# ServiceFoundation/partisan

Measured on AMD Instinct MI355X. Metric: simulated node-rounds/sec (+ msgs/sec), 1M-node HyParView+Plumtree, higher is better.
Workload: dtype u32

## Files before the change

### include/partisan_gpu_sim.h

```cpp
#ifndef PARTISAN_GPU_SIM_H
#define PARTISAN_GPU_SIM_H

#include <stddef.h>
#include <stdint.h>

#ifdef __cplusplus
extern "C" {
#endif

#define PSIM_ABI_VERSION 12

#define PSIM_OK 0
#define PSIM_EINVAL -1
#define PSIM_ENOMEM -2
#define PSIM_EDEVICE -3
#define PSIM_ESTATE -4
#define PSIM_ERANGE -5
#define PSIM_ECOMM -6
#define PSIM_EUNSUPPORTED -7
#define PSIM_ECAPACITY -8

enum psim_msg_type {
    PSIM_MSG_JOIN = 0,
    PSIM_MSG_FORWARD_JOIN = 1,
// ... 309 lines not shown
    uint64_t relays[PSIM_RELAY_CASES];
    uint64_t refused[PSIM_RELAY_CASES];
    uint64_t expired[PSIM_RELAY_CASES];
    uint64_t restarts[PSIM_RELAY_CASES];
    uint64_t in_flight[PSIM_RELAY_CASES];
    uint64_t levels[PSIM_RELAY_CASES];
    uint64_t peak[PSIM_RELAY_CASES];
    uint64_t reserved[8];
} psim_relay_reach;

typedef struct psim_handle psim_handle;

void psim_default_config(psim_config *cfg);
int psim_create(const psim_config *cfg, psim_handle **out);
void psim_destroy(psim_handle *h);
const char *psim_strerror(int code);
int psim_abi_version(void);

int psim_join(psim_handle *h, const uint32_t *nodes, const uint32_t *contacts, size_t n);
int psim_crash(psim_handle *h, const uint32_t *nodes, size_t n);
int psim_revive(psim_handle *h, const uint32_t *nodes, size_t n);
int psim_leave(psim_handle *h, const uint32_t *nodes, size_t n);
int psim_leave_node(psim_handle *h, const uint32_t *actors, const uint32_t *targets, size_t n);
#define PSIM_PARTITION_MAX 254
int psim_set_partition(psim_handle *h, const uint8_t *group, size_t n);
int psim_set_bucket_table(psim_handle *h, const uint8_t *buckets, size_t n);
int psim_set_phash_table(psim_handle *h, const uint32_t *phash, size_t n);
int psim_clear_partition(psim_handle *h);
#define PSIM_OMIT_SEND 0
#define PSIM_OMIT_RECEIVE 1
int psim_set_omission(psim_handle *h, int kind, const uint32_t *src, const uint32_t *dst, size_t n, int on);
int psim_set_faulted(psim_handle *h, const uint32_t *nodes, size_t n, int on);
int psim_clear_faults(psim_handle *h);
int psim_broadcast(psim_handle *h, uint32_t root, uint32_t msg_id);

int psim_step(psim_handle *h, uint32_t n_rounds, psim_round_stats *stats);

int psim_get_nodes(psim_handle *h, uint32_t first, uint32_t count, psim_node_view *out);
int psim_get_round(psim_handle *h, uint64_t *round);
int psim_get_strategy_nodes(psim_handle *h, uint32_t first, uint32_t count, psim_strategy_view *out);
int psim_get_member_bits(psim_handle *h, uint32_t node, uint32_t *words, size_t n_words);
int psim_get_delivery(psim_handle *h, uint32_t first, uint32_t count, uint8_t *have, uint32_t *round,
                      uint32_t *hop);
int psim_get_histograms(psim_handle *h, psim_histograms *out);
int psim_get_strategy_histograms(psim_handle *h, psim_strategy_histograms *out);
int psim_get_graph_metrics(psim_handle *h, const uint32_t *sources, size_t n_sources, uint32_t max_levels,
                           psim_graph_metrics *out);
int psim_get_tree_metrics(psim_handle *h, uint32_t root, uint32_t max_levels, psim_tree_metrics *out);
int psim_get_resilience(psim_handle *h, const psim_failure_case *cases, size_t n_cases, uint64_t fail_seed,
                        uint32_t max_levels, psim_resilience *out);
int psim_get_gossip_reach(psim_handle *h, const psim_gossip_case *cases, size_t n_cases, uint64_t fail_seed,
                          uint32_t max_levels, psim_gossip_reach *out);
int psim_get_relay_reach(psim_handle *h, const psim_relay_case *cases, size_t n_cases, uint32_t max_levels,
                         psim_relay_reach *out);
int psim_snapshot(psim_handle *h, void *buf, size_t cap, size_t *need);
int psim_restore(psim_handle *h, const void *buf, size_t size);

#define PSIM_TRACE_TO   1u
#define PSIM_TRACE_FROM 2u
int psim_trace_watch(psim_handle *h, const uint32_t *nodes, size_t n, uint32_t dir,
                     uint32_t type_mask, size_t capacity);
int psim_trace_read(psim_handle *h, uint32_t *recs, uint32_t *rounds, size_t cap,
                    size_t *n, uint64_t *lost);
int psim_trace_clear(psim_handle *h);

int psim_get_msg_slots(psim_handle *h, uint32_t *ids, uint32_t *roots, size_t cap);

uint32_t psim_xbot_latency(uint64_t seed, uint32_t a, uint32_t b);

typedef struct psim_wire_names {
    const char *prefix;
    const char *host;
    uint32_t ip_base;
    uint32_t port;
} psim_wire_names;
int psim_wire_encode(const uint32_t rec[16], const psim_wire_names *names, uint8_t *buf, size_t cap, size_t *len);
int psim_wire_decode(const uint8_t *buf, size_t len, const psim_wire_names *names, uint32_t dst, uint32_t rec[16],
                     size_t *used);

int psim_record_check(const uint32_t rec[16], const psim_config *cfg);

int psim_debug_kernel_counts(psim_handle *h, uint64_t *out, int cap);

int psim_kernel_times(psim_handle *h, const char **names, double *ms, uint64_t *launches, int cap);

int psim_get_exchange_stats(psim_handle *h, uint64_t *records, uint64_t *bytes);

int psim_comm_id_size(void);
int psim_get_comm_id(void *buf, size_t cap);
int psim_loopback_comm_id(void *buf, size_t cap);

int psim_host_comm_id(void *buf, size_t cap, uint32_t lo, uint32_t hi);
int psim_round_emit(psim_handle *h);
int psim_get_outbound(psim_handle *h, uint32_t *recs, size_t cap, size_t *n);
int psim_round_absorb(psim_handle *h, const uint32_t *recs, size_t n, psim_round_stats *stats);

#ifdef __cplusplus
}
#endif
#endif
```

### partisan_amd/_abi.py

```python
import ctypes as C

import numpy as np

PSIM_ABI_VERSION = 12
PSIM_MAP_BIT = 0x80000000
PSIM_NONE = 0xFFFFFFFF
ACTIVE_CAP, PASSIVE_CAP, IDMAP_CAP = 8, 32, 64
PT_MEMBERS_CAP, PT_SET_POOL, PT_OUT_CAP, EXCHANGE_CAP = 8, 64, 128, 8
PT_ROOTS, MSG_SLOTS = 4, 64
CONN_CAP, CONN_DOWN, CONN_CLOSING = 8, 0x80000000, 0x40000000
OVF_NKINDS = 5
NTYPES = 24
SVIEW_CAP = 128
MANAGER_HYPARVIEW, MANAGER_PLUGGABLE, MANAGER_XBOT = 0, 1, 2
STRATEGY_FULL, STRATEGY_SCAMP_V1, STRATEGY_SCAMP_V2 = 0, 1, 2

MSG_TYPES = [
    "JOIN", "FORWARD_JOIN", "NEIGHBOR", "DISCONNECT", "NEIGHBOR_REQUEST",
    "NEIGHBOR_ACCEPTED", "NEIGHBOR_REJECTED", "SHUFFLE", "SHUFFLE_REPLY",
    "PT_BROADCAST", "PT_PRUNE", "PT_IHAVE", "PT_IGNORED_IHAVE", "PT_GRAFT", "", "",
    "XBOT_OPTIMIZATION", "XBOT_OPTIMIZATION_REPLY", "XBOT_REPLACE", "XBOT_REPLACE_REPLY",
    "XBOT_SWITCH", "XBOT_SWITCH_REPLY",
]
PL_MSG_TYPES = ["HELLO", "STATE", "GOSSIP", "FWD_SUB", "PING", "KEEP_SUB", "REMOVE_SUB", "BOOT_REMOVE"]
# ... 165 lines not shown
class PsimGossipCase(C.Structure):
    _fields_ = [("source", C.c_uint32), ("threshold", C.c_uint32), ("salt", C.c_uint32), ("fanout", C.c_uint32)]


class PsimGossipReach(C.Structure):
    _fields_ = [
        ("n_up", C.c_uint64), ("links", C.c_uint64), ("cases_live", C.c_uint64), ("live_mask", C.c_uint64),
        ("alive", C.c_uint64 * FAIL_CASES), ("reached", C.c_uint64 * FAIL_CASES),
        ("hop_sum", C.c_uint64 * FAIL_CASES), ("ecc", C.c_uint64 * FAIL_CASES),
        ("sent", C.c_uint64 * FAIL_CASES), ("lost", C.c_uint64 * FAIL_CASES),
        ("ecc_max", C.c_uint64), ("levels", C.c_uint64), ("truncated", C.c_uint64),
        ("reserved", C.c_uint64 * 8),
    ]


RELAY_CASES, RELAY_MAX_TTL = 64, 16


class PsimRelayCase(C.Structure):
    _fields_ = [("source", C.c_uint32), ("target", C.c_uint32), ("ttl", C.c_uint32), ("reserved", C.c_uint32)]


class PsimRelayReach(C.Structure):
    _fields_ = [
        ("n_up", C.c_uint64), ("out_entries", C.c_uint64), ("out_usable", C.c_uint64),
        ("out_nonmember", C.c_uint64), ("members_down", C.c_uint64),
        ("out_degree", C.c_uint64 * HIST_BINS),
        ("cases_live", C.c_uint64), ("live_mask", C.c_uint64), ("direct_mask", C.c_uint64),
        ("truncated_mask", C.c_uint64), ("levels_max", C.c_uint64),
        ("delivered", C.c_uint64 * RELAY_CASES), ("first_hop", C.c_uint64 * RELAY_CASES),
        ("hop_sum", C.c_uint64 * RELAY_CASES), ("relays", C.c_uint64 * RELAY_CASES),
        ("refused", C.c_uint64 * RELAY_CASES), ("expired", C.c_uint64 * RELAY_CASES),
        ("restarts", C.c_uint64 * RELAY_CASES), ("in_flight", C.c_uint64 * RELAY_CASES),
        ("levels", C.c_uint64 * RELAY_CASES), ("peak", C.c_uint64 * RELAY_CASES),
        ("reserved", C.c_uint64 * 8),
    ]


NODE_VIEW_DTYPE = np.dtype(PsimNodeView)
STRATEGY_VIEW_DTYPE = np.dtype(PsimStrategyView)
STATS_DTYPE = np.dtype(PsimRoundStats)

_H = C.c_void_p
_P32 = C.POINTER(C.c_uint32)
SIGNATURES = {
    "default_config": (None, [C.POINTER(PsimConfig)]),
    "create": (C.c_int, [C.POINTER(PsimConfig), C.POINTER(C.c_void_p)]),
    "destroy": (None, [_H]),
    "join": (C.c_int, [_H, _P32, _P32, C.c_size_t]),
    "crash": (C.c_int, [_H, _P32, C.c_size_t]),
    "revive": (C.c_int, [_H, _P32, C.c_size_t]),
    "leave": (C.c_int, [_H, _P32, C.c_size_t]),
    "leave_node": (C.c_int, [_H, _P32, _P32, C.c_size_t]),
    "set_partition": (C.c_int, [_H, C.POINTER(C.c_uint8), C.c_size_t]),
    "clear_partition": (C.c_int, [_H]),
    "set_bucket_table": (C.c_int, [_H, C.POINTER(C.c_uint8), C.c_size_t]),
    "set_phash_table": (C.c_int, [_H, _P32, C.c_size_t]),
    "set_omission": (C.c_int, [_H, C.c_int, _P32, _P32, C.c_size_t, C.c_int]),
    "set_faulted": (C.c_int, [_H, _P32, C.c_size_t, C.c_int]),
    "clear_faults": (C.c_int, [_H]),
    "broadcast": (C.c_int, [_H, C.c_uint32, C.c_uint32]),
    "step": (C.c_int, [_H, C.c_uint32, C.POINTER(PsimRoundStats)]),
    "get_nodes": (C.c_int, [_H, C.c_uint32, C.c_uint32, C.POINTER(PsimNodeView)]),
    "get_round": (C.c_int, [_H, C.POINTER(C.c_uint64)]),
    "get_strategy_nodes": (C.c_int, [_H, C.c_uint32, C.c_uint32, C.POINTER(PsimStrategyView)]),
    "get_member_bits": (C.c_int, [_H, C.c_uint32, _P32, C.c_size_t]),
    "get_delivery": (C.c_int, [_H, C.c_uint32, C.c_uint32, C.POINTER(C.c_uint8), _P32, _P32]),
    "get_histograms": (C.c_int, [_H, C.POINTER(PsimHistograms)]),
    "get_msg_slots": (C.c_int, [_H, _P32, _P32, C.c_size_t]),
    "xbot_latency": (C.c_uint32, [C.c_uint64, C.c_uint32, C.c_uint32]),
}
GPU_ONLY = {
    "strerror": (C.c_char_p, [C.c_int]),
    "abi_version": (C.c_int, []),
    "kernel_times": (C.c_int, [_H, C.POINTER(C.c_char_p), C.POINTER(C.c_double),
                               C.POINTER(C.c_uint64), C.c_int]),
    "comm_id_size": (C.c_int, []),
    "get_comm_id": (C.c_int, [C.c_void_p, C.c_size_t]),
    "loopback_comm_id": (C.c_int, [C.c_void_p, C.c_size_t]),
    "snapshot": (C.c_int, [_H, C.c_void_p, C.c_size_t, C.POINTER(C.c_size_t)]),
    "restore": (C.c_int, [_H, C.c_void_p, C.c_size_t]),
    "get_exchange_stats": (C.c_int, [_H, C.POINTER(C.c_uint64), C.POINTER(C.c_uint64)]),
    "debug_kernel_counts": (C.c_int, [_H, C.POINTER(C.c_uint64), C.c_int]),
    "get_strategy_histograms": (C.c_int, [_H, C.POINTER(PsimStrategyHistograms)]),
    "get_graph_metrics": (C.c_int, [_H, _P32, C.c_size_t, C.c_uint32, C.POINTER(PsimGraphMetrics)]),
    "get_tree_metrics": (C.c_int, [_H, C.c_uint32, C.c_uint32, C.POINTER(PsimTreeMetrics)]),
    "get_resilience": (C.c_int, [_H, C.POINTER(PsimFailureCase), C.c_size_t, C.c_uint64, C.c_uint32,
                                 C.POINTER(PsimResilience)]),
    "get_gossip_reach": (C.c_int, [_H, C.POINTER(PsimGossipCase), C.c_size_t, C.c_uint64, C.c_uint32,
                                   C.POINTER(PsimGossipReach)]),
    "get_relay_reach": (C.c_int, [_H, C.POINTER(PsimRelayCase), C.c_size_t, C.c_uint32, C.POINTER(PsimRelayReach)]),
    "trace_watch": (C.c_int, [_H, _P32, C.c_size_t, C.c_uint32, C.c_uint32, C.c_size_t]),
    "trace_read": (C.c_int, [_H, _P32, _P32, C.c_size_t, C.POINTER(C.c_size_t), C.POINTER(C.c_uint64)]),
    "trace_clear": (C.c_int, [_H]),
}
HOST_BOUNDARY = {
    "host_comm_id": (C.c_int, [C.c_void_p, C.c_size_t, C.c_uint32, C.c_uint32]),
    "round_emit": (C.c_int, [_H]),
    "get_outbound": (C.c_int, [_H, _P32, C.c_size_t, C.POINTER(C.c_size_t)]),
    "round_absorb": (C.c_int, [_H, _P32, C.c_size_t, C.POINTER(PsimRoundStats)]),
    "record_check": (C.c_int, [_P32, C.POINTER(PsimConfig)]),
}


def bind(lib, prefix, names):
    out = {}
    for name, (res, args) in names.items():
        fn = getattr(lib, prefix + name)
        fn.restype = res
        fn.argtypes = args
        out[name] = fn
    return out


def u32p(a):
    return a.ctypes.data_as(_P32)
```

### partisan_amd/csrc/psim_consume.hip

```cpp
#include "psim_device.h"
#include "psim_kernels.h"
#include "psim_lite.h"
#include "psim_wave.h"

namespace psim {

#define ID_OF(e, n) (((uint32_t)(e) << 20) | (uint32_t)(n))
#define ID_E(id) ((id) >> 20)
#define ID_C(id) ((id)&0xFFFFFu)

constexpr int WAVES_PER_BLOCK = 4;
#ifndef PSIM_WAVES_PER_SIMD
#define PSIM_WAVES_PER_SIMD 4
#endif

#ifdef PSIM_STAMPS
__device__ unsigned long long g_stamps[32];
__device__ unsigned long long g_stamps_lite[32];
#define STAMP(w, k)                                                                  \
    do {                                                                             \
        uint64_t t_ = __builtin_amdgcn_s_memtime();                                  \
        if (lane_id() == 0) (w).stl[(k)] += t_ - (w).t_last;                         \
        (w).t_last = t_;                                                             \
    } while (0)
// ... 1462 lines not shown
    consume_blocks<false>(args, blockIdx.x, gridDim.x, pool);
}

DEV void body_lite(Wv& w, const NodeIn& x) {
    KArgs& a = kargs();
    const uint32_t l = lane_id();
    w.conn_n = 0; w.conn_dn = 0; w.conn_cl = 0;
    w.work = true;
    st_add(w, ST_PROC, 1);
    STAMP(w, 1);
    for (uint32_t c = 0; c < x.ik; c += 4) {
        uint32_t R4 = inbox_chunk(w, a, x.ib, x.ik, c, x.R0);
        uint32_t cm = x.ik - c < 4 ? x.ik - c : 4;
        for (uint32_t q = 0; q < cm; q++) {
            uint32_t b = q * 16;
            uint32_t tt = rl(R4, b + 2), type = tt & 0xFF;
            if (type >= PSIM_MSG_PT_BROADCAST) continue;
            st_add(w, ST_DELIV + type, 1);
            uint32_t nex = (tt >> 16) & 0xFF;
            uint32_t ex = shfl(R4, (int)((b + 8 + l) & 63));
            ex = l < nex ? ex : 0u;
            const uint32_t p = rl(R4, b + 1), ttl = (tt >> 8) & 0xFF;
            STAMP(w, 2);
            if (type == PSIM_MSG_SHUFFLE_REPLY) {
                merge_exchange(w, ex, nex);
                STAMP(w, 3);
            } else if (ttl > 0 && w.act_n > 1) {
                uint32_t r = select_random(w, w.A, w.act_n, p, w.me, w.me);
                if (r != NONE) hv_send(w, r, PSIM_MSG_SHUFFLE, ttl - 1, 0, 0, ex, nex);
                STAMP(w, 4);
            } else {
                uint32_t RESP = 0;
                uint32_t nr = sublist(w, w.P, w.pas_n, nex, RESP, 0);
                STAMP(w, 5);
                hv_send(w, p, PSIM_MSG_SHUFFLE_REPLY, 0, 0, 0, RESP, nr);
                STAMP(w, 6);
                merge_exchange(w, ex, nex);
                STAMP(w, 7);
            }
        }
    }
    STAMP(w, 2);
    if (x.tf & DESC_SHUFFLE) {
        uint32_t EX;
        uint32_t nex = build_exchange(w, EX);
        uint32_t t = select_random(w, w.A, w.act_n, w.me, w.me, w.me);
        if (t != NONE) hv_send(w, t, PSIM_MSG_SHUFFLE, a.arwl, 0, 0, EX, nex);
        STAMP(w, 8);
    }
}

DEV void writeback_lite(Wv& w) {
    KArgs& a = kargs();
    const uint32_t l = lane_id();
    const size_t li = w.li;
    uint32_t* hrow = reinterpret_cast<uint32_t*>(a.hdr + li);
    const uint32_t k = l & 15;
    const uint32_t hw = k == 0 ? (uint32_t)w.rng : k == 1 ? (uint32_t)(w.rng >> 32)
                      : (w.act_n | (w.pas_n << 8) | (w.sent_n << 16) | (w.sent_head << 24));
    if (l < 16 && (k < 2 || k == 9)) hrow[k] = hw;
    {
        bool dirty = (w.vd & 2u) != 0;
        uint32_t x = shfl(w.P, (int)(l & 31));
        *(dirty ? a.pas + li * PSIM_PASSIVE_CAP + (l & 31) : hrow) = dirty ? x : (uint32_t)w.rng;
    }
    a.ocnt[li] = w.seq;
    st_add(w, ST_BOUND, w.seq > a.obase[li + 1] - w.obase ? 1u : 0u);
    flush_recs(w);
}

#ifndef PSIM_LITE_WAVES
#define PSIM_LITE_WAVES 7
#endif
#ifndef PSIM_LITE_WPB
#define PSIM_LITE_WPB 4
#endif
constexpr uint32_t LITE_WPB = PSIM_LITE_WPB;
__global__ void __launch_bounds__(64 * PSIM_LITE_WPB, PSIM_LITE_WAVES) k_consume_lite(RoundArgs args) {
    if (*kargs().ctl) return;
    __shared__ uint64_t sst[NST];
    __shared__ uint32_t scratch[LITE_WPB][64];
    __shared__ __attribute__((aligned(16))) uint32_t srecs[LITE_WPB][STAGE * 16];
    __shared__ uint32_t skeys[LITE_WPB][STAGE];
    for (int i = threadIdx.x; i < NST; i += blockDim.x) sst[i] = 0;
    __syncthreads();
    const uint32_t wid = threadIdx.x >> 6;
    const uint32_t gw = uni(blockIdx.x * LITE_WPB + wid);
    const uint32_t nw = gridDim.x * LITE_WPB;
    Wv w;
    w.a = &args;
    w.lds = scratch[wid];
    w.nlog = nullptr;
    w.srec = srecs[wid];
    w.skey = skeys[wid];
    w.slots = nullptr;
#ifdef PSIM_STAMPS
    __shared__ uint64_t stamps[LITE_WPB][32];
    if ((threadIdx.x & 63) < 32) stamps[wid][threadIdx.x & 63] = 0;
    w.stl = stamps[wid];
    w.t_last = __builtin_amdgcn_s_memtime();
#endif
    w.st = sst;
    w.round = kargs().round;
    w.SC = 0;
    w.digest = 0;
    w.KM = magic_lanes();
    uint32_t lc[4], na;
    lite_counts(kargs(), lc, na);
    if (gw < na) {
        const uint32_t last = na - 1;
        KArgs& a0 = kargs();
        NodeIn x = load_node<false>(a0, reinterpret_cast<const uint32_t*>(kargs().desc_lite + lite_at(a0, lc, gw))[lane_id() & 3]);
        NodeX y = load_x<true>(kargs(), x);
        NodeIn xn = load_node<false>(kargs(), reinterpret_cast<const uint32_t*>(kargs().desc_lite + lite_at(a0, lc, min(gw + nw, last)))[lane_id() & 3]);
        uint32_t d = reinterpret_cast<const uint32_t*>(kargs().desc_lite + lite_at(a0, lc, min(gw + 2 * nw, last)))[lane_id() & 3];
        for (uint32_t i = gw; i < na; i += nw) {
            STAMP(w, 0);
            begin_node(w, x, y);
            body_lite(w, x);
            NodeX yn = load_x<true>(kargs(), xn);
            STAMP(w, 9);
            writeback_lite(w);
            STAMP(w, 10);
            NodeIn xnn = load_node<false>(kargs(), d);
            d = reinterpret_cast<const uint32_t*>(kargs().desc_lite + lite_at(kargs(), lc, min(i + 3 * nw, last)))[lane_id() & 3];
            x = xn; y = yn; xn = xnn;
            STAMP(w, 11);
        }
    }
#ifdef PSIM_STAMPS
    if (lane_id() < 32) atomicAdd(&g_stamps_lite[lane_id()], (unsigned long long)w.stl[lane_id()]);
#endif
    flush_wave_stats(w, sst);
    __syncthreads();
    for (int i = threadIdx.x; i < NST; i += blockDim.x)
        kargs().stat_lite[(size_t)blockIdx.x * NST + i] = sst[i];
}

struct PtIn {
    uint32_t n, ib, ik, ob, tf;
    uint32_t H, A, R0, CN;
    uint32_t fl, part, oc;
};
struct PtX {
    uint32_t CF, PA, PG, PL;
    uint64_t PO;
};

DEV PtIn load_pt_node(KArgs& a, uint32_t D) {
    const uint32_t l = lane_id();
    PtIn x;
    x.n = rl(D, 0); x.ib = rl(D, 1); x.ik = rl(D, 2) & DESC_CNT_MASK; x.tf = rl(D, 2) >> 28; x.ob = rl(D, 3);
    const size_t li = x.n - a.lo;
    x.H = reinterpret_cast<const uint32_t*>(a.hdr + li)[l & 15];
    x.A = a.act[li * PSIM_ACTIVE_CAP + (l & 7)];
    const uint32_t m = x.ik ? min(l >> 4, x.ik - 1) : 0u;
    x.R0 = reinterpret_cast<const uint32_t*>(a.rec_in + x.ib + m)[l & 15];
    x.CN = a.conn[li * PSIM_CONN_CAP + (l & 7)];
    x.fl = a.flags[x.n];
    x.part = a.part[x.n];
    x.oc = a.ocnt[li];
    return x;
}

DEV uint32_t act_cache(const PtIn& x) {
    const uint32_t l = lane_id(), act_n = rl(x.H, 9) & 0xFF;
    const uint32_t av = shfl(x.A, (int)(l & 7));
    const uint32_t cc = conn_cache_id(x.CN, x.H);
    return l >= 32 && l < 40 && l - 32 < act_n ? av : (l >= 40 ? cc : NONE);
}

DEV PtX load_pt_x(KArgs& a, const PtIn& x) {
    const uint32_t l = lane_id();
    PtX y;
    const size_t li = x.n - a.lo;
    y.CF = cache_flags(a, act_cache(x), x.n);
    y.PA = load_pa(a, li);
    y.PG = a.pt_eag[li * RT_SET + l];
    y.PL = a.pt_laz[li * RT_SET + l];
    y.PO = load_po(a, li, rl(x.H, HW_OUT_EXT));
    return y;
}

DEV void begin_pt(Wv& w, const PtIn& x, const PtX& y) {
    const uint32_t l = lane_id();
    w.li = x.n - kargs().lo;
    w.me = x.n;
    w.rng = ((uint64_t)rl(x.H, 1) << 32) | rl(x.H, 0);
    w.start_round = rl(x.H, 2);
    w.aux = rl(x.H, 5); w.have = rl(x.H, 6); w.trk_round = rl(x.H, 7); w.trk_hop = rl(x.H, 8);
    const uint32_t w10 = rl(x.H, 10);
    w.act_n = rl(x.H, 9) & 0xFF; w.all_n = (w10 >> 16) & 0xFF; w.com_n = w10 >> 24;
    w.out_n = (rl(x.H, 11) >> 16) & 0xFF;
    w.ox = rl(x.H, HW_OUT_EXT);
    w.A = l < PSIM_ACTIVE_CAP ? x.A : 0u;
    w.fl = x.fl;
    w.obase = x.ob;
    w.mypart = x.part;
    w.CV = act_cache(x); w.CF = y.CF;
    const uint32_t w11 = rl(x.H, HW_CONN);
    w.conn_n = w11 & 0xFF; w.conn_dn = (w11 >> 8) & 0xFF; w.conn_cl = w11 >> 24;
    w.CN = l < w.conn_n ? x.CN : 0u;
    load_pt_regs(w, y.PA, y.PG, y.PL, y.PO);
    w.pt_dirty = false;
    w.lazy_quiet = false;
    w.seq = x.oc; w.flushed = x.oc;
}

// ... 105 lines not shown
    __shared__ uint64_t stamps[WAVES_PER_BLOCK][32];
    if ((threadIdx.x & 63) < 32) stamps[wid][threadIdx.x & 63] = 0;
    w.stl = stamps[wid];
    w.t_last = __builtin_amdgcn_s_memtime();
#endif
    w.st = sst;
    w.round = kargs().round;
    w.SC = 0;
    w.digest = 0;
    const uint32_t na = *kargs().n_alist;
    if (gw < na) {
        const uint32_t last = na - 1;
        PtIn x = load_pt_node(kargs(), load_desc(kargs(), gw));
        PtX y = load_pt_x(kargs(), x);
        PtIn xn = load_pt_node(kargs(), load_desc(kargs(), min(gw + nw, last)));
        uint32_t d = load_desc(kargs(), min(gw + 2 * nw, last));
        for (uint32_t i = gw; i < na; i += nw) {
            STAMP(w, 31);
            begin_pt(w, x, y);
            STAMP(w, 29);
            body_pt(w, x);
            PtX yn = load_pt_x(kargs(), xn);
            writeback_pt(w, x.H);
            STAMP(w, 30);
            PtIn xnn = load_pt_node(kargs(), d);
            d = load_desc(kargs(), min(i + 3 * nw, last));
            x = xn; y = yn; xn = xnn;
        }
    }
#ifdef PSIM_STAMPS
    if (lane_id() < 32) atomicAdd(&g_stamps[lane_id()], (unsigned long long)w.stl[lane_id()]);
#endif
    flush_wave_stats(w, sst);
    __syncthreads();
    for (int i = threadIdx.x; i < NST; i += blockDim.x)
        kargs().stat_part[(size_t)blockIdx.x * NST + i] = sst[i];
}

DEV uint64_t relay_emit(KArgs& a, uint64_t slot, uint32_t dst, uint32_t me, uint32_t tt, uint32_t seq,
                        uint32_t a0, uint32_t a1, uint32_t a2, const uint32_t (&X)[8]) {
    const uint32_t W[16] = {dst, me, tt, seq, a0, a1, a2, 0u, X[0], X[1], X[2], X[3], X[4], X[5], X[6], X[7]};
    uint64_t dg = 0;
#pragma unroll
    for (int j = 0; j < 16; j++) dg += (uint64_t)W[j] * digest_mul(j);
    uint4* o = reinterpret_cast<uint4*>(a.rec_out + slot);
    o[0] = make_uint4(dst, me, tt, seq);
    o[1] = make_uint4(a0, a1, a2, 0u);
    if (!PSIM_SHORT_TAIL || ((tt >> 16) & 0xFFu)) {
        o[2] = make_uint4(X[0], X[1], X[2], X[3]);
        o[3] = make_uint4(X[4], X[5], X[6], X[7]);
    }
    a.okey[slot] = dst | (max_emit(tt & 0xFF) << KEY_DST_BITS);
    return dg;
}

DEV void block_append(bool go, const uint4& D, uint4* desc, uint32_t* cnt, uint32_t* wcnt) {
    const uint64_t m = ballot(go);
    const uint32_t wv = threadIdx.x >> 6;
    __syncthreads();
    if (lane_id() == 0) wcnt[wv] = popc(m);
    __syncthreads();
    if (threadIdx.x == 0) {
        uint32_t t = 0;
        for (uint32_t k = 0; k < (blockDim.x >> 6); k++) t += wcnt[k];
        wcnt[4] = t ? atomicAdd(cnt, t) : 0u;
    }
    __syncthreads();
    if (go) {
        uint32_t b0 = wcnt[4];
        for (uint32_t k = 0; k < wv; k++) b0 += wcnt[k];
        desc[b0 + popc(m & lt_mask())] = D;
    }
}

#ifndef PSIM_RELAY_WAVES
#define PSIM_RELAY_WAVES 5
#endif
#ifndef PSIM_RELAY_FJ
#define PSIM_RELAY_FJ 1
#endif
#ifndef PSIM_PTL_BIN
#define PSIM_PTL_BIN 1
#endif
#ifndef PSIM_LITE_BIN
#define PSIM_LITE_BIN 1
#endif
__global__ void __launch_bounds__(256, PSIM_RELAY_WAVES) k_relay(RoundArgs) {
    if (*kargs().ctl) return;
    if (blockIdx.x == 0 && threadIdx.x == 0) kargs().ktime[0] = __builtin_amdgcn_s_memrealtime();
    enum { R_PROC, R_DELIV, R_SHUF, R_FAIL, R_DIGEST, R_BOUND, R_DELIV_FJ, R_FJ, R_N };
    __shared__ unsigned long long sst[R_N];
    __shared__ uint32_t wc5[11][5];
    if (threadIdx.x < R_N) sst[threadIdx.x] = 0;
    __syncthreads();
    const uint32_t l = lane_id();
    const uint32_t na = *kargs().n_alist;
    const uint64_t two58 = 1ull << 58;
    uint32_t v[R_N] = {};
    unsigned long long vdg = 0;
    for (uint32_t base = blockIdx.x * blockDim.x; base < na; base += gridDim.x * blockDim.x) {
        KArgs& a = kargs();
        const uint32_t P = base + threadIdx.x;
        uint4 D = make_uint4(0, 0, 0, 0);
        bool heavy = false, to_pt = false, relay = false, maps = false, shuf = false, lite = false, bcast = false, term = false,
             extra = false;
        Hdr h;
        uint32_t ik = 0, oend = 0;
        uint4 act0 = make_uint4(0, 0, 0, 0), act1 = act0;
        uint32_t me_part = 0;
        uint32_t hvm = 0;
        uint32_t first = 0;
        uint8_t fl0 = 0;
        if (P < na) {
            D = a.desc[P];
            const uint32_t id = D.x, tf = D.z >> 28;
            ik = D.z & DESC_CNT_MASK;
            const size_t li = id - a.lo;
            h = a.hdr[li];
            oend = (uint32_t)a.obase[li + 1];
            const uint4* ar = reinterpret_cast<const uint4*>(a.act + li * PSIM_ACTIVE_CAP);
            act0 = ar[0];
            act1 = ar[1];
            me_part = a.part[id];
            fl0 = a.flags[id];
            uint32_t hvn = 0;
            hvm = 0;
            bool all_relay = true, all_shuf = true, term_out = false, fjn = false;
            uint32_t nf = ~0u;
            bcast = false; term = false; extra = (tf & DESC_SHUFFLE) != 0;
            const uint32_t av[8] = {act0.x, act0.y, act0.z, act0.w, act1.x, act1.y, act1.z, act1.w};
            for (uint32_t j = 0; j < ik; j += 4) {
                uint2 T[4];
#pragma unroll
                for (int q = 0; q < 4; q++) {
                    const uint4 r4 = j + q < ik ? *reinterpret_cast<const uint4*>(a.rec_in + D.y + j + q)
                                                : make_uint4(0, 0, (uint32_t)PSIM_MSG_PT_BROADCAST, 0);
                    T[q] = make_uint2(r4.y, r4.z);
                }
#pragma unroll
                for (int q = 0; q < 4; q++) {
                    const uint32_t tt = T[q].y, type = tt & 0xFF;
                    bcast |= j + q < ik && type == PSIM_MSG_PT_BROADCAST;
                    if (type < PSIM_MSG_PT_BROADCAST || type >= PSIM_MSG_XBOT_OPTIMIZATION) {
                        hvn++;
                        hvm |= j + q < 32 ? 1u << (j + q) : 0u;
                        maps |= type <= PSIM_MSG_NEIGHBOR_ACCEPTED;
                        const uint32_t ttl = (tt >> 8) & 0xFF;
                        const bool relays = ttl > 0 && h.act_n > 1;
                        const bool fj = PSIM_RELAY_FJ && !a.xbot && type == PSIM_MSG_FORWARD_JOIN && ttl > 0 &&
                                        ttl != a.prwl && h.act_n >= 4;
                        fjn |= fj;
                        all_relay &= (type == PSIM_MSG_SHUFFLE && ttl > 0) || fj;
                        all_shuf &= type == PSIM_MSG_SHUFFLE || type == PSIM_MSG_SHUFFLE_REPLY;
                        term |= type == PSIM_MSG_SHUFFLE && !relays;
                        extra |= type == PSIM_MSG_SHUFFLE && relays;
                        nf = type == PSIM_MSG_SHUFFLE && relays ? nf : min(nf, j + q);
                        if (type == PSIM_MSG_SHUFFLE && !relays) {
                            bool in = false;
#pragma unroll
                            for (int k = 0; k < 8; k++) in |= (uint32_t)k < h.act_n && av[k] == T[q].x;
                            term_out |= !in;
                        }
                    }
                }
            }
            const bool fresh = h.start_round == a.round;
            bool exits = false;
            if (a.crash_round) {
                uint32_t cv[PSIM_CONN_CAP] = {};
                if (h.conn_n) {
                    const uint4* cr = reinterpret_cast<const uint4*>(a.conn + li * PSIM_CONN_CAP);
                    const uint4 c0 = cr[0], c1 = cr[1];
                    cv[0] = c0.x; cv[1] = c0.y; cv[2] = c0.z; cv[3] = c0.w;
                    cv[4] = c1.x; cv[5] = c1.y; cv[6] = c1.z; cv[7] = c1.w;
                }
#pragma unroll
                for (int j = 0; j < 8; j++) {
                    bool down = false;
#pragma unroll
                    for (int k = 0; k < PSIM_CONN_CAP; k++) down |= (uint32_t)k < h.conn_n && cv[k] == (av[j] | PSIM_CONN_DOWN);
                    exits |= (uint32_t)j < h.act_n && av[j] != id && av[j] < a.n_nodes && !down &&
                             crashed_now(a, av[j]);
                }
#pragma unroll
                for (int k = 0; k < PSIM_CONN_CAP; k++)
                    exits |= (uint32_t)k < h.conn_n && !(cv[k] & PSIM_CONN_DOWN) && crashed_now(a, cv[k] & KEY_DST_MASK);
            }
            const bool cdown = h.conn_dn != 0 && (hvn > 0 || (tf & DESC_SHUFFLE));
            const bool xwork = a.xbot && (h.conn_cl || (D.z & DESC_XBOT_BIT));
            bool fj_ok = true;
            if (fjn && a.plumtree) {
                const uint4* pr = reinterpret_cast<const uint4*>(a.pt_all + li * PSIM_PT_MEMBERS_CAP);
                const uint4 p0 = pr[0], p1 = pr[1];
                const uint32_t pv[8] = {p0.x, p0.y, p0.z, p0.w, p1.x, p1.y, p1.z, p1.w};
                fj_ok = h.all_n == h.act_n;
#pragma unroll
                for (int j = 0; j < 8; j++) {
                    bool in = false;
#pragma unroll
                    for (int k = 0; k < 8; k++) in |= (uint32_t)k < h.all_n && pv[k] == av[j];
                    fj_ok &= (uint32_t)j >= h.act_n || in;
                }
            }
            heavy = exits || fresh || ((tf & DESC_PROMO) && h.act_n < a.min_active) ||
                    (hvn && !all_shuf && !(all_relay && fj_ok)) || term_out || cdown || xwork;
            lite = !heavy && hvn && !(all_relay && h.act_n > 1);
            first = a.relay_lead && lite && ik <= 32 && nf < ik ? nf : 0u;
            shuf = !heavy && !lite && (tf & DESC_SHUFFLE);
            maps = maps || exits || (tf & DESC_PROMO) || h.conn_cl;
            relay = !heavy && !lite && hvn > 0;
            const bool pt_msgs = !fresh && ik > hvn, origin = (tf & DESC_ORIGIN) != 0;
            const bool lazy = (tf & DESC_LAZY) && h.out_n > 0;
            to_pt = a.plumtree && (pt_msgs || origin || lazy);
            if (!heavy && !lite && (relay || to_pt || shuf)) v[R_PROC]++;
        }
        uint32_t upm[4] = {NONE, NONE, NONE, NONE};
        if (P < na && (relay || lite)) {
            const uint32_t av[8] = {act0.x, act0.y, act0.z, act0.w, act1.x, act1.y, act1.z, act1.w};
            KArgs& a = kargs();
#pragma unroll
            for (int j = 0; j < 8; j += 2) {
                const uint32_t q0 = (uint32_t)j < h.act_n && av[j] < a.n_nodes ? av[j] : D.x;
                const uint32_t q1 = (uint32_t)j + 1 < h.act_n && av[j + 1] < a.n_nodes ? av[j + 1] : D.x;
                upm[j >> 1] = (uint32_t)a.upart[q0] | ((uint32_t)a.upart[q1] << 16);
            }
        }
        const bool origin_node = ((D.z >> 28) & DESC_ORIGIN) != 0;
        {
            const bool ptl = P < na && to_pt && !origin_node, lt = P < na && lite;
            const bool pe = ptl && (!a.ptl_split || (!heavy && !lite && !shuf)), pl = ptl && !pe;
            const bool pb = bcast || !PSIM_PTL_BIN;
            const bool lt0 = lt && !(extra && PSIM_LITE_BIN), lt1 = lt && extra && PSIM_LITE_BIN;
            const bool tb = term || !PSIM_LITE_BIN;
            const bool g[11] = {P < na && heavy, P < na && to_pt && origin_node, pe && pb,
                                P < na && shuf, lt0 && tb, pe && !pb, lt0 && !tb,
                                lt1 && tb, lt1 && !tb, pl && pb, pl && !pb};
            uint64_t m[11];
#pragma unroll
            for (int k = 0; k < 11; k++) m[k] = ballot(g[k]);
            const uint32_t wv = threadIdx.x >> 6, nwv = blockDim.x >> 6;
            __syncthreads();
            if (l == 0)
#pragma unroll
                for (int k = 0; k < 11; k++) wc5[k][wv] = popc(m[k]);
            __syncthreads();
            if (threadIdx.x < 11) {
                const uint32_t k = threadIdx.x;
                uint32_t t = 0;
                for (uint32_t j = 0; j < nwv; j++) t += wc5[k][j];
                uint32_t* cnt = k == 0 ? a.n_slow : k == 1 ? a.n_pt : k == 2 ? a.n_ptl : k == 3 ? a.n_shuf
                              : k == 4 ? a.n_lite : k == 5 ? a.n_ptl + 1 : k < 9 ? a.n_lite + (k - 5)
                              : a.n_ptl + (k - 7);
                wc5[k][4] = t ? atomicAdd(cnt, t) : 0u;
            }
            __syncthreads();
#pragma unroll
            for (int k = 0; k < 11; k++)
                if (g[k]) {
                    uint32_t b0 = wc5[k][4];
                    for (uint32_t j = 0; j < wv; j++) b0 += wc5[k][j];
                    const uint32_t at = b0 + popc(m[k] & lt_mask());
                    uint4* desc = k == 0 ? a.desc_slow : k == 1 ? a.desc_pt : k == 2 || k == 5 || k >= 9 ? a.desc_ptl
                                : k == 3 ? a.desc_shuf : a.desc_lite;
                    const uint32_t nl = a.n_local;
                    desc[k == 5 || k == 6 ? nl - 1 - at : k == 7 || k == 9 ? nl + at
                         : k == 8 || k == 10 ? 2 * nl - 1 - at : at] =
                        k == 0 && maps ? make_uint4(D.x, D.y, D.z | DESC_MAPS_BIT, D.w)
                        : k == 4 || (k >= 6 && k <= 8) ? make_uint4(D.x, D.y + first, D.z - first, D.w) : D;
                }
        }
        if (P >= na || heavy) continue;
        const uint32_t id = D.x;
        const size_t li = id - a.lo;
        const uint32_t A[8] = {act0.x, act0.y, act0.z, act0.w, act1.x, act1.y, act1.z, act1.w};
        uint64_t rng = h.rng;
        uint32_t seq = 0;
        uint32_t cm = 0;
#pragma unroll
        for (int j = 0; j < 8; j++)
            cm |= ((upm[j >> 1] >> (16 * (j & 1))) & 0xFFFFu) == me_part ? 1u << j : 0u;
        const bool big = ik > 32;
        uint32_t rm = relay ? hvm : hvm & ((1u << first) - 1u);
        for (uint32_t jr = 0; big ? relay && jr < ik : rm != 0; jr++) {
            if (!big) {
                jr = (uint32_t)__ffs(rm) - 1;
                rm &= rm - 1;
            }
            const Msg* rp = a.rec_in + D.y + jr;
            const uint32_t tt = rp->tt;
            if ((tt & 0xFF) >= PSIM_MSG_PT_BROADCAST) continue;
            const bool fj = (tt & 0xFF) == PSIM_MSG_FORWARD_JOIN;
            const uint32_t ttl = (tt >> 8) & 0xFF, nex = (tt >> 16) & 0xFF, src = rp->src;
            const uint32_t jq = fj ? rp->a0 : NONE, jpe = fj ? rp->a1 : 0u;
            v[R_DELIV] += fj ? 0u : 1u;
            v[R_DELIV_FJ] += fj ? 1u : 0u;
            uint32_t elig = 0;
#pragma unroll
            for (int j = 0; j < 8; j++)
                elig |= (j < h.act_n && A[j] != src && A[j] != id && A[j] != jq) ? (1u << j) : 0u;
            const uint32_t cnt = __popc(elig);
            if (cnt) {
                uint32_t k;
                for (;;) {
                    const uint64_t x = draw58_at(rng++, id, a.seed);
                    if (x < cnt) { k = (uint32_t)x; break; }
                    const uint32_t i = mod_small(x, cnt);
                    if (x - i <= two58 - cnt) { k = i; break; }
                }
                uint32_t e = elig;
                for (uint32_t j = 0; j < k; j++) e &= e - 1;
                const uint32_t jr_ = (uint32_t)__ffs(e) - 1;
                const uint32_t r = A[jr_];
                if (r < a.n_nodes && ((cm >> jr_) & 1u)) {
                    rng++;
                    uint32_t X[8] = {};
                    if (!fj) {
                        const uint4* ex = reinterpret_cast<const uint4*>(rp->ex);
                        const uint4 e0 = ex[0], e1 = ex[1];
                        const uint32_t E[8] = {e0.x, e0.y, e0.z, e0.w, e1.x, e1.y, e1.z, e1.w};
#pragma unroll
                        for (int j = 0; j < 8; j++) X[j] = (uint32_t)j < nex ? E[j] : 0u;
                    }
                    vdg += relay_emit(a, D.w + seq, r, id,
                                              fj ? PSIM_MSG_FORWARD_JOIN | ((ttl - 1) << 8)
                                                 : PSIM_MSG_SHUFFLE | ((ttl - 1) << 8) | (nex << 16),
                                              seq, fj ? jq : 0u, jpe, 0u, X);
                    seq++;
                    v[R_SHUF] += fj ? 0u : 1u;
                    v[R_FJ] += fj ? 1u : 0u;
                } else {
                    v[R_FAIL]++;
                }
            }
        }
        if (rng != h.rng) a.hdr[li].rng = rng;
        if (lite) {
            a.lite_cm[li] = (uint16_t)(cm | (seq << 8));
            continue;
        }
        a.ocnt[li] = seq;
        v[R_BOUND] += seq > oend - D.w ? 1u : 0u;
        if (!to_pt) {
            a.flags[id] = (uint8_t)((fl0 & (F_UP | F_CRASHED)) | (h.out_n ? F_LAZY : 0) |
                                    (min((uint32_t)h.out_n, 15u) << F_OUTN_SHIFT) |
                                    (h.act_n < a.min_active ? F_LOWACT : 0));
        }
    }
#pragma unroll
    for (int k = 0; k < R_N; k++) {
        unsigned long long t = k == R_DIGEST ? vdg : (unsigned long long)v[k];
        for (uint32_t o = 32; o > 0; o >>= 1) {
            const int from = (int)(((threadIdx.x & 63u) ^ o) << 2);
// ... 825 lines not shown
```

### partisan_amd/csrc/psim_engine.hip

```cpp
#include <hip/hip_runtime.h>
#include <rccl/rccl.h>

#include <algorithm>
#include <chrono>
#include <cstdio>
#include <cstdlib>
#include <cstring>
#include <new>
#include <set>
#include <vector>

#include "psim_host.h"
#include "psim_payload.h"
#include "psim_wave.h"

using namespace psim;

namespace {

constexpr uint32_t PREP_BLK = 1024;
#ifndef PSIM_PREP_NPT
#define PSIM_PREP_NPT 4
#endif
constexpr uint32_t PREP_NPT = PSIM_PREP_NPT;
// ... 1185 lines not shown
    uint32_t* sv = reinterpret_cast<uint32_t*>(mk);
    uint32_t* ll = sv + RUN_LDS;
    for (uint32_t dl = threadIdx.x; dl < W; dl += blockDim.x) {
        const uint32_t k = cnt[dl];
        if (k < 2) continue;
        if (k > RUN_SHORT) {
            ll[atomicAdd(&s_nl, 1u)] = dl;
            continue;
        }
        uint32_t* q = ix + pre[dl];
        uint32_t v[RUN_SHORT];
#pragma unroll
        for (uint32_t t = 0; t < RUN_SHORT; t++) v[t] = t < k ? q[t] : 0xFFFFFFFFu;
#pragma unroll
        for (uint32_t r = 0; r < RUN_SHORT; r++) {
#pragma unroll
            for (uint32_t t = r & 1; t + 1 < RUN_SHORT; t += 2) {
                const uint32_t lo_ = v[t], hi_ = v[t + 1];
                v[t] = min(lo_, hi_);
                v[t + 1] = max(lo_, hi_);
            }
        }
#pragma unroll
        for (uint32_t t = 0; t < RUN_SHORT; t++)
            if (t < k) q[t] = v[t];
    }
    __syncthreads();
    if (prep) {
        const uint32_t nrb = max(1u, W >> rp.pshift), c = threadIdx.x & 63;
        for (uint32_t j = threadIdx.x >> 6; j < nrb; j += blockDim.x >> 6) {
            const uint32_t R = ((b << wshift) >> rp.pshift) + j;
            if (R >= rp.nranges) break;
            const uint64_t up = s_rp[j][RP_UP], ws = s_rp[j][RP_W], qp = s_rp[j][RP_QP];
            const unsigned long long bsum = *reinterpret_cast<const unsigned long long*>(&s_rp[j][RP_BLO]);
            if (c == 0) {
                rp.tiles[R] = ((uint64_t)bsum << 32) + ws;
                rp.btot[R] = bsum;
                if (R == rp.nranges - 1) rp.tiles[rp.nranges] = 0;
            }
            if (c < NST)
                rp.part[(size_t)R * NST + c] = c == ST_UP ? up : c == ST_DROPPED ? (uint64_t)s_rp[j][RP_DROP]
                                             : c == ST_PROC ? qp : c == ST_FAIL ? (uint64_t)s_rp[j][RP_QF]
                                             : c == ST_BYTES ? ws * (2 * NODE_STATE_BYTES) : 0ull;
        }
    }
    const uint32_t nl = s_nl, wv = threadIdx.x >> 6, nwv = blockDim.x >> 6;
    for (uint32_t q = wv; q < nl; q += nwv) {
        const uint32_t dl = ll[q], k = cnt[dl];
        if (k <= 64) wave_sort64(ix + pre[dl], k);
    }
    __syncthreads();
    for (uint32_t q = 0; q < nl; q++) {
        const uint32_t dl = ll[q], k = cnt[dl];
        if (k > 64) sort_run_block(ix + pre[dl], k, tmp + s0 + pre[dl], sv);
    }
    __syncthreads();
    const uint32_t m4 = (s1 - s0) * 4, bd = blockDim.x;
    for (uint32_t t = threadIdx.x; t < m4; t += 2 * bd) {
        const uint32_t t2 = t + bd;
        uint4 a, c = make_uint4(0, 0, 0, 0);
        if (WIRE) {
            a = wire_piece(heads, tails, ix[t >> 2], t & 3);
            if (t2 < m4) c = wire_piece(heads, tails, ix[t2 >> 2], t2 & 3);
        } else {
            a = rec_piece(rec, ix[t >> 2], t & 3);
            if (t2 < m4) c = rec_piece(rec, ix[t2 >> 2], t2 & 3);
        }
        reinterpret_cast<uint4*>(&inbox[s0 + (t >> 2)])[t & 3] = a;
        if (t2 < m4) reinterpret_cast<uint4*>(&inbox[s0 + (t2 >> 2)])[t2 & 3] = c;
    }
}

__global__ void __launch_bounds__(BLK) k_node_prep(RoundArgs a, const unsigned long long* bmask, uint64_t* packed,
                                                   uint64_t* part, uint32_t* ocnt, unsigned long long* btot,
                                                   uint32_t per, uint64_t* tiles, uint32_t* gcnt, uint32_t ngcnt) {
    if (*a.ctl) return;
    for (uint32_t j = blockIdx.x * blockDim.x + threadIdx.x; j < ngcnt; j += gridDim.x * blockDim.x) gcnt[j] = 0;
    if (gcnt && blockIdx.x == 0 && threadIdx.x == 0) const_cast<uint32_t*>(a.ctl)[2] = 0;
    __shared__ unsigned long long s_up, s_drop, s_b, s_w, s_qp, s_qf;
    if (threadIdx.x == 0) { s_up = 0; s_drop = 0; s_b = 0; s_w = 0; s_qp = 0; s_qf = 0; }
    if (blockIdx.x == 0 && threadIdx.x == 0) {
        a.ktime[0] = ~0ull; a.ktime[1] = 0; *a.n_slow = 0; *a.n_pt = 0;
        if (a.n_shuf) *a.n_shuf = 0;
        if (a.n_lite) { a.n_lite[0] = 0; a.n_lite[1] = 0; a.n_lite[2] = 0; a.n_lite[3] = 0; }
        if (a.n_ptl) { a.n_ptl[0] = 0; a.n_ptl[1] = 0; a.n_ptl[2] = 0; a.n_ptl[3] = 0; }
        if (a.n_stop) *a.n_stop = 0;
    }
    __syncthreads();
    if (a.upart && a.upart_dirty)
        for (uint32_t g = blockIdx.x * blockDim.x + threadIdx.x; g < a.n_nodes; g += gridDim.x * blockDim.x)
            a.upart[g] = (a.flags[g] & F_UP) ? (upart_t)a.part[g] : UPART_DOWN;
    PrepSums ps{0, 0, 0, 0, 0, 0};
#ifdef PSIM_BOUND_TERMS
    unsigned long long bt[BT_N] = {};
#endif
    const uint32_t i0 = blockIdx.x * per, i1 = min(a.n_local, i0 + per);
    struct PrepIn {
        uint8_t f;
        unsigned long long cbi;
        uint32_t st, org;
        unsigned long long bm;
    };
    auto prep_in = [&](uint32_t i) {
        PrepIn q{0, 0ull, 0u, 0u, 0ull};
        if (i < i1) {
            q.f = a.flags[a.lo + i];
            q.cbi = a.in_cb[i];
            q.st = a.start[i];
            q.org = a.pl ? 0u : a.origin[i];
            q.bm = a.pl ? 0ull : bmask[i];
        }
        return q;
    };
    auto node = [&](uint32_t i, const PrepIn& cur) -> uint64_t {
        if (!a.pl) return hv_node_prep<true>(a, i, cur.f, cur.cbi, cur.bm, cur.st, cur.org, ps BT_ARG);
        uint64_t b = 0;
        uint32_t w = 0;
        const uint32_t c = (uint32_t)cur.cbi;
        if (cur.f & F_UP) {
            const uint32_t st = cur.st, r = a.round;
            const Hdr& x = a.hdr[i];
            bool pending = x.join_contact != PSIM_NONE;
            bool per = due(a.periodic, r, st);
            bool leave = x.pad1[0] != 0;
            if (a.strategy == PSIM_STRATEGY_FULL)
                b = a.fanout ? (uint64_t)c + a.fanout + 1
                             : ((uint64_t)c + 2 + (leave ? 1 : 0)) * (a.n_nodes + 1);
            else
            {
                const uint64_t vn = x.act_n, vg = vn + c + 1;
                b = (uint64_t)c + (pending ? 1 + 2 * vg : 0) + (per ? 1 + vg : 0) + (leave ? vn : 0) + 1;
            }
            w = c > 0 || (pending && !x.have) || per || leave;
            ps.up++;
        } else {
            ps.drop += c;
        }
        ps.bs += b;
        ps.ws += w;
        BTERM(BT_TOTAL, b);
        return (b << 32) | w;
    };
    PrepIn q[PREP_CHUNK], qn[PREP_CHUNK];
    const uint32_t cstep = PREP_CHUNK * blockDim.x;
#pragma unroll
    for (uint32_t k = 0; k < PREP_CHUNK; k++) q[k] = prep_in(i0 + threadIdx.x + k * blockDim.x);
    for (uint32_t c0 = i0 + threadIdx.x; c0 < i1; c0 += cstep) {
        uint64_t pk[PREP_CHUNK];
#pragma unroll
        for (uint32_t k = 0; k < PREP_CHUNK; k++) {
            const uint32_t i = c0 + k * blockDim.x;
            pk[k] = i < i1 ? node(i, q[k]) : 0ull;
        }
#pragma unroll
        for (uint32_t k = 0; k < PREP_CHUNK; k++) qn[k] = prep_in(c0 + cstep + k * blockDim.x);
#pragma unroll
        for (uint32_t k = 0; k < PREP_CHUNK; k++) {
            const uint32_t i = c0 + k * blockDim.x;
            if (i < i1) {
                packed[i] = pk[k];
                ocnt[i] = 0;
            }
        }
#pragma unroll
        for (uint32_t k = 0; k < PREP_CHUNK; k++) q[k] = qn[k];
    }
#ifdef PSIM_BOUND_TERMS
// ... 27 lines not shown
    }
    if (threadIdx.x == 0) btot[blockIdx.x] = s_b;
    if (threadIdx.x < NST) {
        uint64_t v = threadIdx.x == ST_UP ? s_up : threadIdx.x == ST_DROPPED ? s_drop : threadIdx.x == ST_PROC ? s_qp
                   : threadIdx.x == ST_FAIL ? s_qf : threadIdx.x == ST_BYTES && !a.pl ? s_w * (2 * NODE_STATE_BYTES)
                   : 0ull;
        part[(size_t)blockIdx.x * NST + threadIdx.x] = v;
    }
}

struct DescIn {
    uint32_t in_beg, cnt, start, origin;
};
__device__ __forceinline__ DescIn desc_in(const RoundArgs& a, uint32_t li, uint64_t pk,
                                          const uint32_t* __restrict__ in_beg,
                                          const unsigned long long* __restrict__ cb,
                                          const uint32_t* __restrict__ start) {
    DescIn d{0, 0, 0, 0};
    if (pk & 1u) {
        d.in_beg = in_beg[li];
        d.cnt = (uint32_t)cb[li];
        d.start = start[li];
        d.origin = a.plumtree && !a.pl ? a.origin[li] : 0u;
    }
    return d;
}

__device__ __forceinline__ void desc_entry(const RoundArgs& a, uint32_t li, uint64_t P, uint64_t pk, const DescIn& d,
                                           uint4* __restrict__ desc, uint64_t* __restrict__ obase, uint32_t* nact,
                                           unsigned long long tot, uint64_t* hout, uint64_t cap, uint32_t* ctl) {
    obase[li] = P >> 32;
    if (li == a.n_local) {
        *nact = (uint32_t)P;
        obase[li] = tot;
        hout[PIN_TOTAL] = tot;
        if (tot > hout[PIN_TMAX]) hout[PIN_TMAX] = tot;
        if (cap && tot + 1 > cap) { ctl[1] = a.round; __threadfence(); ctl[0] = 1; }
        return;
    }
    if (!(pk & 1u)) return;
    if (d.cnt > DESC_CNT_MASK) hout[PIN_BIGIN] = 1;
    const uint32_t st = d.start, r = a.round;
    const uint32_t tf = (a.random_promotion && due(a.promotion_period, r, st) ? DESC_PROMO : 0u) |
                        (due(a.shuffle_period, r, st) ? DESC_SHUFFLE : 0u) |
                        (a.plumtree && due(a.lazy_tick_period, r, st) ? DESC_LAZY : 0u) |
                        (d.origin ? DESC_ORIGIN : 0u);
    const uint32_t xb = a.xbot && due(a.xbot_period, r, st) ? DESC_XBOT_BIT : 0u;
    desc[(uint32_t)P] = make_uint4(a.lo + li, d.in_beg, d.cnt | xb | (tf << 28), (uint32_t)(P >> 32));
}

__device__ unsigned long long btot_sum(const unsigned long long* btot, uint32_t nbt) {
    __shared__ unsigned long long s_w[PREP_BLK / 64], s_tot;
    unsigned long long t = 0;
    for (uint32_t j = threadIdx.x; j < nbt; j += blockDim.x) t += btot[j];
    for (int o = 32; o > 0; o >>= 1) t += __shfl_xor(t, o);
    if ((threadIdx.x & 63) == 0) s_w[threadIdx.x >> 6] = t;
    __syncthreads();
    if (threadIdx.x == 0) {
        unsigned long long u = 0;
        for (uint32_t k = 0; k < blockDim.x / 64; k++) u += s_w[k];
        s_tot = u;
    }
    __syncthreads();
    return s_tot;
}


__global__ void __launch_bounds__(PREP_BLK) k_desc(const uint64_t* __restrict__ packed,
                                                  const uint64_t* __restrict__ tiles, uint32_t per,
                                                  const uint32_t* __restrict__ in_beg,
                                                  const unsigned long long* __restrict__ cb,
                                                  const uint32_t* __restrict__ start, RoundArgs a,
                                                  uint4* __restrict__ desc, uint64_t* __restrict__ obase,
                                                  uint32_t* nact, const unsigned long long* btot,
                                                  uint32_t nranges, uint64_t* hout, uint64_t cap, uint32_t* ctl,
                                                  uint32_t* gcnt, uint32_t ngcnt) {
    if (*ctl) return;
    if (gcnt) {
        for (uint32_t j = blockIdx.x * blockDim.x + threadIdx.x; j < ngcnt; j += gridDim.x * blockDim.x) gcnt[j] = 0;
        if (blockIdx.x == 0 && threadIdx.x == 0) {
            ctl[2] = 0;
            a.ktime[0] = ~0ull; a.ktime[1] = 0; *a.n_slow = 0; *a.n_pt = 0;
            if (a.n_shuf) *a.n_shuf = 0;
            if (a.n_lite) { a.n_lite[0] = 0; a.n_lite[1] = 0; a.n_lite[2] = 0; a.n_lite[3] = 0; }
            if (a.n_ptl) { a.n_ptl[0] = 0; a.n_ptl[1] = 0; a.n_ptl[2] = 0; a.n_ptl[3] = 0; }
            if (a.n_stop) *a.n_stop = 0;
        }
    }
    const bool last = blockIdx.x == gridDim.x - 1;
    const uint32_t r0 = blockIdx.x * DESC_RANGES;
    const uint32_t i0 = r0 * per, i1 = min(a.n_local, i0 + DESC_RANGES * per);
    uint64_t tp = 0;
#pragma unroll
    for (uint32_t k = 0; k < DESC_RANGES; k++) {
        const uint32_t j = threadIdx.x + k * PREP_BLK;
        tp += j < r0 ? tiles[j] : 0ull;
    }
    uint32_t li = i0 + threadIdx.x;
    uint64_t pk = li < i1 ? packed[li] : 0ull;
    DescIn d = desc_in(a, li, pk, in_beg, cb, start);
    const unsigned long long tot = last ? btot_sum(btot, nranges) : 0ull;
    uint64_t carry;
    (void)block_excl<uint64_t, PREP_BLK>(tp, &carry);
    for (uint32_t k = i0; k < i1; k += PREP_BLK) {
        if (k != i0) {
            li = k + threadIdx.x;
            pk = li < i1 ? packed[li] : 0ull;
            d = desc_in(a, li, pk, in_beg, cb, start);
        }
        uint64_t pass;
        const uint64_t e = block_excl<uint64_t, PREP_BLK>(pk, &pass);
        if (li < i1) desc_entry(a, li, carry + e, pk, d, desc, obase, nact, 0ull, hout, cap, ctl);
        carry += pass;
    }
    if (last && threadIdx.x == 0)
        desc_entry(a, a.n_local, carry, 0ull, DescIn{0, 0, 0, 0}, desc, obase, nact, tot, hout, cap, ctl);
}

constexpr uint32_t TR_BLK = 1024;
constexpr uint32_t TR_SPAN = 2048;
constexpr uint32_t TR_WAVES = TR_BLK / 64;

struct TraceWatch {
    const uint32_t* bits;
    uint32_t n_nodes, dir, type_mask;
};

DEV bool trace_watched(const TraceWatch& w, uint32_t id) {
    return !w.bits || (id < w.n_nodes && ((w.bits[id >> 5] >> (id & 31u)) & 1u));
}

__global__ void __launch_bounds__(TR_BLK) k_trace_count(const Msg* __restrict__ inbox, uint32_t m, uint32_t span,
                                                        TraceWatch w, uint32_t* __restrict__ cnt,
                                                        unsigned long long* __restrict__ ballots) {
    __shared__ uint32_t wc[TR_WAVES];
    const uint64_t base = (uint64_t)blockIdx.x * span;
    uint32_t c = 0;
    for (uint32_t off = threadIdx.x; off < span; off += TR_BLK) {
        const uint64_t i = base + off;
        bool hit = false;
        if (i < m) {
            const uint4 hd = *reinterpret_cast<const uint4*>(inbox + i);
            const uint32_t t = hd.z & 0xFFu;
            hit = t < 32u && ((w.type_mask >> t) & 1u) &&
                  (((w.dir & PSIM_TRACE_TO) && trace_watched(w, hd.x)) ||
                   ((w.dir & PSIM_TRACE_FROM) && trace_watched(w, hd.y)));
        }
        const uint64_t b = ballot(hit);
        if (lane_id() == 0) ballots[i >> 6] = b;
        c += popc(b);
    }
    if (lane_id() == 0) wc[threadIdx.x >> 6] = c;
    __syncthreads();
    if (threadIdx.x == 0) {
        uint32_t t = 0;
        for (uint32_t k = 0; k < TR_WAVES; k++) t += wc[k];
        cnt[blockIdx.x] = t;
    }
}

__global__ void __launch_bounds__(TR_BLK) k_trace_copy(const Msg* __restrict__ inbox, uint32_t span,
                                                       const uint32_t* __restrict__ cnt,
                                                       const unsigned long long* __restrict__ ballots,
                                                       const unsigned long long* __restrict__ tot_in,
                                                       unsigned long long* __restrict__ tot_out,
                                                       Msg* __restrict__ out, uint32_t* __restrict__ rounds,
                                                       unsigned long long cap, uint32_t round) {
    __shared__ uint32_t wsum[TR_WAVES], wc[TR_WAVES];
    __shared__ uint8_t sel[TR_WAVES][64];
    const uint32_t l = lane_id(), wv = threadIdx.x >> 6;
    const uint32_t mine = wave_sum(threadIdx.x < blockIdx.x ? cnt[threadIdx.x] : 0u);
    if (l == 0) wsum[wv] = mine;
    __syncthreads();
    unsigned long long rank0 = tot_in[0];
    for (uint32_t k = 0; k < TR_WAVES; k++) rank0 += wsum[k];
    const uint64_t base = (uint64_t)blockIdx.x * span;
    for (uint32_t p0 = 0; p0 < span; p0 += TR_BLK) {
        const uint32_t off = p0 + wv * 64u;
        const uint64_t g0 = base + off;
        const uint64_t b = off < span ? ballots[g0 >> 6] : 0ull;
        const uint32_t nb = popc(b);
        if ((b >> l) & 1u) sel[wv][popc(b & ((1ull << l) - 1ull))] = (uint8_t)l;
        if (l == 0) wc[wv] = nb;
        __syncthreads();
        unsigned long long r = rank0;
        uint32_t pass = 0;
        for (uint32_t k = 0; k < TR_WAVES; k++) {
            r += k < wv ? wc[k] : 0u;
            pass += wc[k];
        }
        for (uint32_t q = l >> 2; q < nb; q += 16u) {
            const unsigned long long at = r + q;
            if (at < cap) {
                const uint4* sp = reinterpret_cast<const uint4*>(inbox + g0 + sel[wv][q]);
                reinterpret_cast<uint4*>(out + at)[l & 3u] = sp[l & 3u];
                if ((l & 3u) == 0) rounds[at] = round;
            }
        }
        rank0 += pass;
        __syncthreads();
    }
    if (blockIdx.x == gridDim.x - 1 && threadIdx.x == 0) tot_out[0] = rank0;
}

const char* kKernName[KT_N] = {"events", "prepare", "consume", "scan", "compact", "sort",
                               "exchange", "gather", "stats", "k_host_export", "k_host_import", "pay_pack",
                               "k_trace_count", "k_trace_copy"};

constexpr uint64_t RESERVE_PER_NODE = 24;
constexpr uint64_t RCAP_PER_NODE = 4;
constexpr uint64_t RCAP_RESERVE = 8;
constexpr double RCAP_FREE_FRAC = 0.30;
constexpr double OUTBOX_SPARE = 0.12;

inline bool local_route(const psim_handle* h) { return h->G == 1 && !h->ranked; }

inline bool ships_rows(const psim_handle* h) { return h->fw != 0 && h->G > 1 && !h->hosted; }

constexpr int PTL_EARLY_DEFAULT = 0;
int ptl_early_knob() {
    static const int v = [] {
        const char* e = getenv("PSIM_PTL_EARLY");
        const int x = e && *e ? atoi(e) : -1;
        return x >= 0 && x <= 2 ? x : PTL_EARLY_DEFAULT;
    }();
    return v;
}

constexpr int RELAY_LEAD_DEFAULT = 1;
bool relay_lead_knob() {
    static const bool v = [] {
        const char* e = getenv("PSIM_RELAY_LEAD");
        return e && *e ? atoi(e) != 0 : RELAY_LEAD_DEFAULT != 0;
    }();
    return v;
}

constexpr int PREP_FUSED_DEFAULT = 1;
bool prep_fused_knob() {
#ifdef PSIM_BOUND_TERMS
    return false;
#else
    static const bool v = [] {
        const char* e = getenv("PSIM_PREP_FUSED");
        return e && *e ? atoi(e) != 0 : PREP_FUSED_DEFAULT != 0;
    }();
    return v;
#endif
}

uint32_t route_wshift(uint32_t n) {
    uint32_t wshift = n > (1u << 26) ? 13 : n > (1u << 22) ? 12 : 11;
    static const int env = getenv("PSIM_ROUTE_WSHIFT") ? atoi(getenv("PSIM_ROUTE_WSHIFT")) : 0;
    if (env >= (int)WSHIFT_MIN && env <= (int)WSHIFT_MAX) wshift = (uint32_t)env;
    return wshift;
}

bool prep_fused_handle(const psim_handle* h, const Shard* s) {
    return prep_fused_knob() && h->G == 1 && !h->ranked && h->route_fused && s->n <= (1u << 26) &&
           h->cfg.manager != PSIM_MANAGER_PLUGGABLE;
}

RoundArgs make_args(psim_handle* h, Shard* s) {
    RoundArgs a;
    memset(&a, 0, sizeof a);
    const psim_config& c = h->cfg;
    a.n_nodes = h->N; a.round = (uint32_t)h->round; a.seed = c.seed;
    a.lo = s->lo; a.n_local = s->n;
    a.max_active = c.max_active_size; a.min_active = c.min_active_size;
    a.max_passive = c.max_passive_size; a.arwl = c.arwl; a.prwl = c.prwl;
    a.k_active = c.k_active; a.k_passive = c.k_passive;
    a.shuffle_period = c.shuffle_period; a.promotion_period = c.promotion_period;
    a.random_promotion = c.random_promotion; a.plumtree = c.plumtree;
    a.lazy_tick_period = c.lazy_tick_period;
    a.tracked_msg = h->tracked_msg;
    a.origin = s->origin.p;
    a.slots = s->slots.p;
    a.flags = s->flags.p; a.part = s->part.p; a.hdr = s->hdr.p; a.crash_bits = s->crash_bits.p;
    a.upart = s->upart.p;
    a.lite_cm = s->lite_cm.p;
    a.btab = h->btab ? s->btab.p : nullptr;
    a.act = s->act.p; a.pas = s->pas.p; a.sentm = s->sentm.p; a.recvm = s->recvm.p;
    a.mapx = s->mapx.p; a.mapx_top = s->mapx_top.p;
    a.mapx_rows = (uint32_t)(s->mapx.n / IDMAP_EXT);
    a.pt_all = s->pt_all.p; a.pt_com = s->pt_com.p; a.pt_eag = s->pt_eag.p; a.pt_laz = s->pt_laz.p;
    a.pt_rt = s->pt_rt.p;
    a.pt_out = s->pt_out.p; a.outx = s->outx.p; a.outx_top = s->outx_top.p;
    a.conn = s->conn.p;
    a.outx_rows = (uint32_t)(s->outx.n / OUT_EXT);
    a.start = s->start.p;
    a.pl = c.manager == PSIM_MANAGER_PLUGGABLE;
    a.xbot = c.manager == PSIM_MANAGER_XBOT; a.xbot_period = c.xbot_period;
    a.ptl_split = ptl_early_knob() != 0;
    a.relay_lead = relay_lead_knob() && h->lite.kernel != psim::k_consume_lite;
    a.strategy = c.strategy; a.periodic = c.periodic_interval; a.scamp_c = c.scamp_c;
    a.fanout = c.fanout; a.fw = h->fw; a.tomb = h->tomb;
    a.fbits = s->fbits.p; a.sview = s->sview.p; a.sinv = s->sinv.p;
    a.ktime = reinterpret_cast<unsigned long long*>(s->stat_out.p + NST);
    a.ctl = s->ctl.p;
    a.desc_slow = s->desc_slow.p; a.n_slow = s->n_slow.p;
    a.desc_pt = s->desc_pt.p; a.n_pt = s->n_pt.p;
    a.desc_shuf = s->desc_shuf.p; a.n_shuf = s->n_shuf.p;
    a.desc_lite = s->desc_lite.p; a.n_lite = s->n_lite.p;
    a.desc_ptl = s->desc_ptl.p; a.n_ptl = s->n_ptl.p;
    a.stop_ids = s->stop_ids.p; a.n_stop = s->n_stop.p;
    a.faults = h->faults; a.n_omit_s = h->n_omit_s; a.n_omit_r = h->n_omit_r;
    a.faulted = s->faulted.p; a.omit = s->omit.p;
    return a;
}

int route_buffers(Shard* s, bool both_inboxes);

struct KTimer {
    Shard* s;
    int slot;
    KTimer(psim_handle* h, Shard* s_, int k) : s(s_), slot(-1) {
        if (!h->phase_timers || s->tn >= Shard::MAXT) return;
        slot = s->tn++;
        s->tk[slot] = k;
        (void)hipEventRecord(s->ev[slot][0], s->stream);
    }
    ~KTimer() {
        if (slot >= 0) (void)hipEventRecord(s->ev[slot][1], s->stream);
    }
};

void flush_timers(psim_handle* h, Shard* s) {
    for (int i = 0; i < s->tn; i++) {
        float ms = 0;
        if (hipEventElapsedTime(&ms, s->ev[i][0], s->ev[i][1]) != hipSuccess) continue;
        h->kt_ms[s->tk[i]] += ms;
        h->kt_n[s->tk[i]]++;
    }
    s->tn = 0;
}

int scan_desc(Shard* s, const RoundArgs& a, bool resets = false) {
    k_desc<<<(s->pgrid + DESC_RANGES - 1) / DESC_RANGES, PREP_BLK, 0, s->stream>>>(
        s->bound.p, s->pscan.p, s->pper, s->in_beg.p, s->cb.p, s->start.p, a, s->desc.p, s->obase.p, s->d_nact.p,
        s->btot.p, s->pgrid, s->pin_dev, s->desc_cap, s->ctl.p, resets ? s->gcnt.p : nullptr,
        resets ? (uint32_t)s->gcnt.n : 0u);
    HIP_TRY(hipGetLastError());
    return PSIM_OK;
}

int stream_wait(Shard* s) {
    HIP_TRY(hipEventRecord(s->wait_ev, s->stream));
    hipError_t e;
    while ((e = hipEventQuery(s->wait_ev)) == hipErrorNotReady) {
    }
    if (e != hipSuccess) {
        static bool said = false;
        if (!said) std::fprintf(stderr, "psim: event query: %s; synchronising\n", hipGetErrorString(e));
        said = true;
        HIP_TRY(hipStreamSynchronize(s->stream));
    }
    return PSIM_OK;
}

template <typename T>
T read1(Shard* s, const T* p) {
    T v{};
    (void)hipMemcpyAsync(&v, p, sizeof(T), hipMemcpyDeviceToHost, s->stream);
    (void)stream_wait(s);
    return v;
}

int upload(Shard* s, DBuf<uint32_t>& b, const std::vector<uint32_t>& v) {
    TRY(b.ensure(v.size()));
    HIP_TRY(hipMemcpyAsync(b.p, v.data(), v.size() * 4, hipMemcpyHostToDevice, s->stream));
    return PSIM_OK;
}

struct RoundCtl {
    bool crashes = false;
    uint64_t bcast_clear = 0;
};
// ... 675 lines not shown
    if (!h->pend_b_root.empty()) {
        for (size_t i = 0; i < h->pend_b_root.size(); i++) {
            const uint32_t k = h->pend_b_msg[i] % PSIM_MSG_SLOTS;
            ctl.bcast_clear |= 1ull << k;
            h->slot_tab[k] = h->pend_b_msg[i];
            h->slot_tab[PSIM_MSG_SLOTS + k] = h->pend_b_root[i] | PSIM_MAP_BIT;
        }
        h->tracked_msg = h->pend_b_msg.back();
    }
}

int round_front(psim_handle* h, bool events_applied, bool from_partition) {
    RoundCtl ctl;
    ctl.crashes = !h->pend_crash.empty();
    if (!events_applied) bcast_slots(h, ctl);
    if (h->faults_dirty) {
        if (h->nx_faulted.size() != h->N) h->nx_faulted.assign(h->N, 0);
        h->n_omit_s = (uint32_t)h->nx_omit_s.size();
        h->n_omit_r = (uint32_t)h->nx_omit_r.size();
        h->faults = h->n_omit_s || h->n_omit_r || h->nx_nfaulted;
    }
    for (Shard* s : h->shards) s->tn = 0;
    std::vector<RoundArgs> args(h->shards.size());
    for (size_t i = 0; i < h->shards.size() && !from_partition; i++)
        TRY(phase_events_prepare(h, h->shards[i], ctl, args[i], !events_applied, false, events_applied));
    static const long long fail_round = getenv("PSIM_TEST_FAIL_ROUND") ? atoll(getenv("PSIM_TEST_FAIL_ROUND")) : -1;
    if (fail_round >= 0 && h->round == (uint64_t)fail_round) {
        for (Shard* s : h->shards) (void)hipStreamSynchronize(s->stream);
        return PSIM_ENOMEM;
    }
    for (size_t i = 0; i < h->shards.size() && !from_partition; i++) TRY(phase_consume(h, h->shards[i], args[i]));
    return PSIM_OK;
}

int round_back(psim_handle* h, uint64_t* st);

int run_round(psim_handle* h, uint64_t* st, bool events_applied = false, bool from_partition = false) {
    TRY(round_front(h, events_applied, from_partition));
    if (local_route(h)) {
        TRY(phase_route_local(h, h->shards[0]));
    } else {
        for (Shard* s : h->shards) TRY(phase_partition(h, s));
        if (h->ranked) TRY(exchange_rccl(h));
        else TRY(exchange_local(h));
    }
    return round_back(h, st);
}

int round_back(psim_handle* h, uint64_t* st) {
    for (Shard* s : h->shards) {
        TRY(phase_stats(h, s, h->pend_crash));
        if (!h->pend_b_root.empty())
            k_origin<<<grid_for(h->pend_b_root.size()), BLK, 0, s->stream>>>(
                s->origin.p, s->lo, s->n, s->bc_roots.p, s->bc_msgs.p, (uint32_t)h->pend_b_root.size(), s->flags.p,
                true, s->ctl.p);
    }
    memset(st, 0, NST * 8);
    for (Shard* s : h->shards) {
        TRY(stream_wait(s));
        flush_timers(h, s);
        for (int k = 0; k < NST; k++) st[k] += s->pin[k];
        if (local_route(h) && s->pin[PIN_OVF]) {
            const uint64_t m = s->pin[PIN_OVF];
            s->pin[PIN_OVF] = 0;
            if (s->rcap < m + m / 2) {
                const uint64_t want = m + m / 2;
                if (want <= (1ull << 26)) while (s->rcap < want) s->rcap <<= 1;
                else s->rcap = (want + (1ull << 20) - 1) >> 20 << 20;
            }
            TRY(route_buffers(s, false));
            TRY(phase_route_local(h, s, true));
            TRY(stream_wait(s));
        }
        if (local_route(h)) s->m_in = (uint32_t)s->pin[PIN_M];
        if (h->ranked) xcaps_update(h, s, s->pin);
        static const bool trace_relay = getenv("PSIM_TRACE_RELAY") != nullptr;
        if (trace_relay && s->rgrid)
        {
            uint64_t em = 0;
            for (int k = 0; k < ST_NTYPES; k++) em += s->pin[ST_EMIT + k];
            std::fprintf(stderr, "psim: round %llu shard %u: %u nodes with work, %u to k_consume, %u to k_pt, "
                         "%u to k_shuf, %u to k_consume_lite, %u to k_ptl, outbox bound %llu, emitted %llu\n",
                         (unsigned long long)h->round, s->idx, read1(s, s->d_nact.p), read1(s, s->n_slow.p),
                         read1(s, s->n_pt.p), read1(s, s->n_shuf.p), read1(s, s->n_lite.p) + read1(s, s->n_lite.p + 1) + read1(s, s->n_lite.p + 2) + read1(s, s->n_lite.p + 3),
                         read1(s, s->n_ptl.p) + read1(s, s->n_ptl.p + 1) + read1(s, s->n_ptl.p + 2) + read1(s, s->n_ptl.p + 3),
                         (unsigned long long)s->pin[PIN_TOTAL], (unsigned long long)em);
        }
        if (s->pin[NST] != ~0ull && s->pin[NST + 1] > s->pin[NST]) {
            h->kt_ms[KT_CONSUME] += (double)(s->pin[NST + 1] - s->pin[NST]) * 1e-5;
            h->kt_n[KT_CONSUME]++;
        }
    }
    if (st[ST_BOUND]) {
        std::fprintf(stderr, "psim: round %llu: %llu nodes emitted past their outbox bound (engine bug)\n",
                     (unsigned long long)h->round, (unsigned long long)st[ST_BOUND]);
        return PSIM_EDEVICE;
    }
    for (uint32_t j : h->pend_join) h->pend_join_mark[j] = 0;
    h->pend_crash.clear(); h->pend_join.clear(); h->pend_contact.clear();
    h->pend_lv_a.clear(); h->pend_lv_t.clear();
    if (st[ST_STOP]) {
        std::vector<uint32_t> ids;
        for (Shard* s : h->shards) {
            const size_t k = read1(s, s->n_stop.p);
            if (!k) continue;
            const size_t at = ids.size();
            ids.resize(at + k);
            HIP_TRY(hipMemcpyAsync(ids.data() + at, s->stop_ids.p, k * 4, hipMemcpyDeviceToHost, s->stream));
            TRY(stream_wait(s));
        }
        if (h->ranked) {
            Shard* s = h->shards[0];
            const uint32_t W = h->world;
            std::vector<uint64_t> cnt(W), mine(ids.begin(), ids.end());
            const uint64_t k = mine.size();
            TRY(h->comm_cnt.ensure(W + 1));
            HIP_TRY(hipMemcpyAsync(h->comm_cnt.p + W, &k, 8, hipMemcpyHostToDevice, s->stream));
            TRY(h->comm->all_gather(h->comm_cnt.p + W, h->comm_cnt.p, 8, s->stream));
            HIP_TRY(hipMemcpyAsync(cnt.data(), h->comm_cnt.p, W * 8, hipMemcpyDeviceToHost, s->stream));
            TRY(stream_wait(s));
            const uint64_t mk = *std::max_element(cnt.begin(), cnt.end());
            mine.resize(mk, 0);
            std::vector<uint64_t> all((size_t)W * mk);
            TRY(h->comm_cnt.ensure((size_t)W * mk + mk));
            HIP_TRY(hipMemcpyAsync(h->comm_cnt.p + (size_t)W * mk, mine.data(), mk * 8, hipMemcpyHostToDevice,
                                   s->stream));
            TRY(h->comm->all_gather(h->comm_cnt.p + (size_t)W * mk, h->comm_cnt.p, mk * 8, s->stream));
            HIP_TRY(hipMemcpyAsync(all.data(), h->comm_cnt.p, all.size() * 8, hipMemcpyDeviceToHost, s->stream));
            TRY(stream_wait(s));
            ids.clear();
            for (uint32_t r = 0; r < W; r++)
                for (uint64_t j = 0; j < cnt[r]; j++) ids.push_back((uint32_t)all[(size_t)r * mk + j]);
        }
        std::sort(ids.begin(), ids.end());
        h->pend_crash.insert(h->pend_crash.end(), ids.begin(), ids.end());
    }
    h->pend_part_set = h->pend_part_clear = false;
    h->faults_dirty = false;
    h->pend_b_root.clear(); h->pend_b_msg.clear();
    h->round++;
    return PSIM_OK;
}

void fill_stats(const uint64_t* s, uint64_t round, psim_round_stats* o) {
    memset(o, 0, sizeof *o);
    o->round = round;
    for (int i = 0; i < ST_NTYPES; i++) {
        o->emitted[i] = s[ST_EMIT + i];
        o->delivered[i] = s[ST_DELIV + i];
    }
    o->dropped = s[ST_DROPPED]; o->nodes_up = s[ST_UP]; o->nodes_processed = s[ST_PROC];
    o->exits = s[ST_EXITS]; o->send_fail = s[ST_FAIL]; o->first_deliveries = s[ST_FIRST];
    o->overflow = s[ST_OVF]; o->digest = s[ST_DIGEST]; o->state_bytes = s[ST_BYTES];
    for (int k = 0; k < PSIM_OVF_NKINDS; k++) o->overflow_by[k] = s[ST_OVF_BY + k];
    o->omitted = s[ST_OMIT];
}

void pending_swap(psim_handle* h, PendingEvents& e) {
    std::swap(h->pend_crash, e.crash); std::swap(h->pend_join, e.join); std::swap(h->pend_contact, e.contact);
    std::swap(h->pend_join_mark, e.join_mark);
    std::swap(h->pend_lv_a, e.lv_a); std::swap(h->pend_lv_t, e.lv_t);
    std::swap(h->pend_part, e.part);
    std::swap(h->pend_part_set, e.part_set); std::swap(h->pend_part_clear, e.part_clear);
    std::swap(h->pend_b_root, e.b_root); std::swap(h->pend_b_msg, e.b_msg);
    std::swap(h->faults_dirty, e.faults_dirty);
}

// ... 375 lines not shown
    }
    if (done > 0) {
        for (uint32_t j : h->pend_join) h->pend_join_mark[j] = 0;
        h->pend_crash.clear(); h->pend_join.clear(); h->pend_contact.clear();
        h->pend_part_set = h->pend_part_clear = false;
        h->pend_b_root.clear(); h->pend_b_msg.clear();
        h->faults_dirty = false;
    }
    s->m_in = (uint32_t)s->pin[PIN_M];
    *done_out = done;
    if (done == nb) {
        h->round = r0 + nb;
        s->xbatch = std::min<uint32_t>(2 * s->xbatch, BATCH_MAX);
        return PSIM_OK;
    }
    s->xbatch = std::max<uint32_t>(2, s->xbatch / 4);
    HIP_TRY(hipMemsetAsync(s->ctl.p, 0, sizeof cw, s->stream));
    h->round = r0 + done;
    const bool short_outbox = cw[0] == 1 && cw[1] == (uint32_t)h->round;
    uint64_t st[NST];
    if (short_outbox) {
        std::fprintf(stderr, "psim: round %llu: outbox grows past its capacity (%zu -> %llu slots)\n",
                     (unsigned long long)h->round, s->outbox.n, (unsigned long long)s->pin[PIN_TOTAL] + 1);
        TRY(stream_wait(s));
    }
    TRY(run_round(h, st, done == 0, !short_outbox));
    if (st_out) fill_stats(st, r0 + done, &st_out[done]);
    *done_out = done + 1;
    return PSIM_OK;
}

int shard_alloc(psim_handle* h, Shard* s) {
    HIP_TRY(hipStreamCreateWithFlags(&s->stream, hipStreamNonBlocking));
    HIP_TRY(hipEventCreateWithFlags(&s->wait_ev, hipEventDisableTiming));
    for (int k = 0; k < 2; k++) {
        HIP_TRY(hipStreamCreateWithFlags(&s->side[k], hipStreamNonBlocking));
        HIP_TRY(hipEventCreateWithFlags(&s->join_ev[k], hipEventDisableTiming));
    }
    HIP_TRY(hipEventCreateWithFlags(&s->fork_ev, hipEventDisableTiming));
    if (s->n > (1u << 26)) {
        HIP_TRY(hipFuncSetAttribute((const void*)k_bucket_route<false>, hipFuncAttributeMaxDynamicSharedMemorySize,
                                    8192 * 16));
        HIP_TRY(hipFuncSetAttribute((const void*)k_bucket_route<true>, hipFuncAttributeMaxDynamicSharedMemorySize,
                                    8192 * 16));
    }
    HIP_TRY(hipHostMalloc((void**)&s->pin, (size_t)PIN_STRIDE * (1 + BATCH_MAX) * sizeof(uint64_t), hipHostMallocMapped));
    HIP_TRY(hipHostGetDevicePointer((void**)&s->pin_dev, s->pin, 0));
    memset(s->pin, 0, (size_t)PIN_STRIDE * (1 + BATCH_MAX) * sizeof(uint64_t));
    for (int k = 0; k < Shard::MAXT; k++) {
        HIP_TRY(hipEventCreate(&s->ev[k][0]));
        HIP_TRY(hipEventCreate(&s->ev[k][1]));
    }
    s->ev_live = true;
    const size_t N = h->N, n = std::max<uint32_t>(s->n, 1);
    int rc = 0;
    rc |= s->flags.alloc(N); rc |= s->part.alloc(N); rc |= s->hdr.alloc(n);
    if (h->cfg.manager != PSIM_MANAGER_PLUGGABLE) { rc |= s->upart.alloc(N); rc |= s->lite_cm.alloc(n); }
    rc |= s->crash_bits.alloc((N >> (CRASH_GRAIN_SHIFT + 5)) + 1);
    rc |= s->act.alloc(n * PSIM_ACTIVE_CAP); rc |= s->pas.alloc(n * PSIM_PASSIVE_CAP);
    rc |= s->sentm.alloc(n * IDMAP_IN); rc |= s->recvm.alloc(n * IDMAP_IN);
    if (h->cfg.manager != PSIM_MANAGER_PLUGGABLE) {
        const size_t rows = h->cfg.manager == PSIM_MANAGER_XBOT ? 2 * n : std::max<size_t>(1024, n / 32);
        rc |= s->mapx.alloc(rows * IDMAP_EXT);
    }
    rc |= s->mapx_top.alloc(1);
    rc |= s->pt_all.alloc(n * PSIM_PT_MEMBERS_CAP); rc |= s->pt_com.alloc(n * PSIM_PT_MEMBERS_CAP);
    rc |= s->pt_eag.alloc(n * RT_SET); rc |= s->pt_laz.alloc(n * RT_SET); rc |= s->pt_rt.alloc(n * RT_WORDS);
    rc |= s->origin.alloc(n); rc |= s->slots.alloc(2 * PSIM_MSG_SLOTS);
    rc |= s->pt_out.alloc(n * OUT_IN); rc |= s->start.alloc(n);
    if (h->cfg.manager != PSIM_MANAGER_PLUGGABLE) rc |= s->conn.alloc(n * PSIM_CONN_CAP);
    if (h->cfg.manager != PSIM_MANAGER_PLUGGABLE) {
        size_t rows = std::max<size_t>(1024, n / 8);
        if (const char* e = getenv("PSIM_OUTX_ROWS")) rows = std::max<size_t>(1, (size_t)atoll(e));
        rc |= s->outx.alloc(rows * OUT_EXT);
    }
    rc |= s->outx_top.alloc(1);
    rc |= s->ocnt.alloc(n); rc |= s->cb.alloc(n + 1);
    rc |= s->in_beg.alloc(n + 1); rc |= s->bound.alloc(n + 1); rc |= s->pscan.alloc(4097); rc |= s->obase.alloc(n + 1);
    rc |= s->bmask.alloc(n); rc |= s->btot.alloc(4096);
    rc |= s->desc.alloc(n); rc |= s->d_nact.alloc(1);
    rc |= s->desc_slow.alloc(n); rc |= s->n_slow.alloc(1);
    rc |= s->desc_pt.alloc(n); rc |= s->n_pt.alloc(1);
    rc |= s->desc_shuf.alloc(n); rc |= s->n_shuf.alloc(1);
    rc |= s->desc_lite.alloc(2 * n); rc |= s->n_lite.alloc(4);
    rc |= s->desc_ptl.alloc(2 * n); rc |= s->n_ptl.alloc(4);
    if (h->cfg.manager == PSIM_MANAGER_PLUGGABLE) { rc |= s->stop_ids.alloc(n); rc |= s->n_stop.alloc(1); }
    rc |= s->stat_out.alloc(STAT_OUT_N);
    rc |= s->ctl.alloc(4);
    rc |= s->stat_tile.alloc((size_t)STAT_TILES * NST);
    rc |= s->ikeys.alloc(1024); rc |= s->ivals.alloc(1024);
    rc |= s->recvh.alloc(1024); rc |= s->recvt.alloc(1024); rc |= s->wseg.alloc(130); rc |= s->inbox.alloc(1024); rc |= s->outbox.alloc(1024);
    if (h->cfg.manager == PSIM_MANAGER_PLUGGABLE) {
        if (h->cfg.strategy == PSIM_STRATEGY_FULL) {
            rc |= s->fbits.alloc(n * 2 * h->fw);
            rc |= s->pay_top.alloc(1);
            rc |= s->pay[0].alloc(2 * h->fw); rc |= s->pay[1].alloc(2 * h->fw);
        } else {
            rc |= s->sview.alloc(n * PSIM_SVIEW_CAP);
            if (h->cfg.strategy == PSIM_STRATEGY_SCAMP_V2) rc |= s->sinv.alloc(n * PSIM_SVIEW_CAP);
        }
    }
    if (rc) return PSIM_ENOMEM;
    HIP_TRY(hipDeviceSynchronize());
    return PSIM_OK;
}

void trace_release(Shard* s) {
    s->tr_bits.release(); s->tr_round.release(); s->tr_cnt.release(); s->tr_rec.release();
    s->tr_tot.release(); s->tr_ballot.release();
    s->tr_cur = 0;
}

void shard_free(Shard* s) {
    if (s->stream) (void)hipStreamSynchronize(s->stream);
    s->flags.release(); s->part.release(); s->upart.release(); s->lite_cm.release(); s->hdr.release(); s->crash_bits.release(); s->btab.release();
    s->act.release(); s->pas.release(); s->sentm.release(); s->recvm.release();
    s->pt_all.release(); s->pt_com.release();
    s->mapx.release(); s->mapx_top.release();
    s->pt_eag.release(); s->pt_laz.release(); s->pt_out.release(); s->start.release(); s->conn.release();
    s->outx.release(); s->outx_top.release();
    s->pt_rt.release(); s->origin.release(); s->slots.release(); s->bc_roots.release(); s->bc_msgs.release();
    s->ikeys.release(); s->ivals.release(); s->recvh.release(); s->recvt.release(); s->wseg.release(); s->inbox.release();
    if (s->pin) (void)hipHostFree(s->pin);
    if (s->wait_ev) (void)hipEventDestroy(s->wait_ev);
    s->wait_ev = nullptr;
    for (int k = 0; k < 2; k++) {
        if (s->join_ev[k]) (void)hipEventDestroy(s->join_ev[k]);
        if (s->side[k]) (void)hipStreamDestroy(s->side[k]);
        s->join_ev[k] = nullptr;
        s->side[k] = nullptr;
    }
    if (s->fork_ev) (void)hipEventDestroy(s->fork_ev);
    s->fork_ev = nullptr;
    s->pin = nullptr;
    s->outbox.release(); s->okey.release(); s->ocnt.release();
    s->cb.release(); s->in_beg.release();
    s->rank.release(); s->bmask.release(); s->btot.release();
    s->hist.release(); s->hoff.release(); s->rtot.release(); s->rbase.release(); s->pairs.release(); s->tmp.release();
    s->stop_ids.release(); s->n_stop.release();
    s->desc.release(); s->d_nact.release(); s->desc_slow.release(); s->n_slow.release(); s->desc_pt.release(); s->n_pt.release(); s->desc_shuf.release(); s->n_shuf.release(); s->desc_lite.release(); s->n_lite.release(); s->desc_ptl.release(); s->n_ptl.release(); s->bound.release(); s->pscan.release();
    s->obase.release(); s->stat_part.release(); s->stat_out.release(); s->stat_tile.release(); s->d_off.release();
    s->cub_tmp.release(); s->ev_ids.release(); s->ev_contacts.release(); s->sendbuf.release(); s->ctl.release();
    s->sview.release(); s->sinv.release(); s->fbits.release(); s->pay[0].release(); s->pay[1].release();
    s->pay_top.release();
    s->pbits.release(); s->prank.release(); s->plist.release(); s->paysend.release(); s->pay_imp.release(); s->pcnt_d.release();
    trace_release(s);
    if (s->ev_live)
        for (int k = 0; k < Shard::MAXT; k++) {
            (void)hipEventDestroy(s->ev[k][0]);
            (void)hipEventDestroy(s->ev[k][1]);
        }
    if (s->stream) (void)hipStreamDestroy(s->stream);
    delete s;
}

const char kHostMagic[8] = {'P', 'S', 'I', 'M', 'H', 'O', 'S', 'T'};
bool host_id_range(const void* id, uint32_t* lo, uint32_t* hi) {
    if (!id || memcmp(id, kHostMagic, sizeof kHostMagic) != 0) return false;
    memcpy(lo, (const char*)id + sizeof kHostMagic, 4);
    memcpy(hi, (const char*)id + sizeof kHostMagic + 4, 4);
    return *lo < *hi;
}

}

extern "C" {

// ... 946 lines not shown
        HIP_TRY(hipMemcpy(rd.data() + at, s->tr_round.p, stored[k] * 4, hipMemcpyDeviceToHost));
        at += stored[k];
    }
    std::vector<size_t> ord(all.size());
    for (size_t i = 0; i < ord.size(); i++) ord[i] = i;
    auto before = [&](size_t a, size_t b) {
        if (rd[a] != rd[b]) return rd[a] < rd[b];
        const Msg &x = all[a], &y = all[b];
        if (x.dst != y.dst) return x.dst < y.dst;
        if (x.src != y.src) return x.src < y.src;
        return x.seq < y.seq;
    };
    if (!std::is_sorted(ord.begin(), ord.end(), before)) std::stable_sort(ord.begin(), ord.end(), before);
    const bool pl = h->cfg.manager == PSIM_MANAGER_PLUGGABLE;
    for (size_t i = 0; i < kept; i++) {
        uint32_t* o = recs + i * 16;
        memcpy(o, &all[ord[i]], sizeof(Msg));
        const uint32_t t = o[2] & 0xFFu;
        if (pl && !(h->fw && (t == PSIM_PL_STATE || t == PSIM_PL_GOSSIP))) o[7] = 0;
        rounds[i] = rd[ord[i]];
    }
    for (Shard* s : h->shards) {
        HIP_TRY(hipMemsetAsync(s->tr_tot.p, 0, 2 * sizeof(unsigned long long), s->stream));
        HIP_TRY(hipStreamSynchronize(s->stream));
    }
    return PSIM_OK;
}

int psim_trace_clear(psim_handle* h) {
    if (!h) return PSIM_EINVAL;
    if (!h->trace_on) return PSIM_OK;
    if (hipSetDevice(h->device) != hipSuccess) return PSIM_EDEVICE;
    for (Shard* s : h->shards) {
        (void)hipStreamSynchronize(s->stream);
        trace_release(s);
    }
    h->trace_on = false;
    return PSIM_OK;
}

int psim_get_exchange_stats(psim_handle* h, uint64_t* records, uint64_t* bytes) {
    if (!h || !records || !bytes) return PSIM_EINVAL;
    *records = h->x_records;
    *bytes = h->x_bytes;
    return PSIM_OK;
}

int psim_kernel_times(psim_handle* h, const char** names, double* ms, uint64_t* launches, int cap) {
    if (!h) return PSIM_EINVAL;
    int k = 0;
    for (; k < KT_N && k < cap; k++) {
        if (names) names[k] = kKernName[k];
        if (ms) ms[k] = h->kt_ms[k];
        if (launches) launches[k] = h->kt_n[k];
    }
    return k;
}

int psim_debug_kernel_counts(psim_handle* h, uint64_t* out, int cap) {
    if (!h || !out || cap < 24) return PSIM_EINVAL;
    if (h->cfg.manager == PSIM_MANAGER_PLUGGABLE) return 0;
    Shard* s = h->shards[0];
    const uint32_t rows = s->pgrid + s->cgrid + s->rgrid + s->tgrid + s->sgrid + s->lgrid + s->qgrid + s->egrid;
    std::vector<uint64_t> st((size_t)rows * NST);
    HIP_TRY(hipStreamSynchronize(s->stream));
    HIP_TRY(hipMemcpy(st.data(), s->stat_part.p, st.size() * 8, hipMemcpyDeviceToHost));
    const uint32_t b_cons = s->pgrid, b_rel = b_cons + s->cgrid, b_pt = b_rel + s->rgrid, b_sh = b_pt + s->tgrid,
                   b_li = b_sh + s->sgrid, b_pl = b_li + s->lgrid, b_ple = b_pl + s->qgrid, b_end = b_ple + s->egrid;
    const uint32_t rng[8][2] = {{b_rel, b_pt}, {b_sh, b_li}, {b_li, b_pl}, {b_cons, b_rel}, {b_pl, b_end}, {b_pt, b_sh},
                                {0, b_cons}, {b_ple, b_end}};
    const int nk = cap >= 32 ? 8 : cap >= 28 ? 7 : 6;
    for (int k = 0; k < nk; k++) {
        uint64_t v[3] = {0, 0, 0};
        for (uint32_t r = rng[k][0]; r < rng[k][1]; r++) {
            const uint64_t* row = st.data() + (size_t)r * NST;
            v[0] += row[ST_PROC];
            for (int t = 0; t < ST_NTYPES; t++) { v[1] += row[ST_DELIV + t]; v[2] += row[ST_EMIT + t]; }
        }
        out[4 * k] = v[0]; out[4 * k + 1] = v[1]; out[4 * k + 2] = v[2]; out[4 * k + 3] = 0;
    }
    return nk;
}

int psim_debug_stamps(unsigned long long* out, int cap) {
    if (!out || cap < 96) return PSIM_EINVAL;
    return psim::debug_stamps(out);
}

int psim_comm_id_size(void) { return (int)sizeof(ncclUniqueId); }

int psim_loopback_comm_id(void* buf, size_t cap) { return psim::loopback_new_id(buf, cap); }

int psim_get_comm_id(void* buf, size_t cap) {
    if (!buf || cap < sizeof(ncclUniqueId)) return PSIM_EINVAL;
    ncclUniqueId id;
    if (ncclGetUniqueId(&id) != ncclSuccess) return PSIM_ECOMM;
    memcpy(buf, &id, sizeof id);
    return PSIM_OK;
}

}
```

### partisan_amd/csrc/psim_kernels.h

```cpp
#pragma once
#include <stddef.h>

#include "psim_device.h"

namespace psim {

#ifndef PSIM_UPART8
#define PSIM_UPART8 1
#endif
#if PSIM_UPART8
typedef uint8_t upart_t;
#else
typedef uint16_t upart_t;
#endif

struct RoundArgs {
    uint32_t n_nodes, round;
    uint32_t lo, n_local;
    uint64_t seed;
    uint32_t max_active, min_active, max_passive, arwl, prwl, k_active, k_passive;
    uint32_t shuffle_period, promotion_period, random_promotion, plumtree, lazy_tick_period;
    uint32_t xbot, xbot_period;
    uint32_t ptl_split;
    uint32_t relay_lead;
    uint32_t crash_round, tracked_msg;
    uint32_t upart_dirty;
    uint32_t lazy_wake;
    uint8_t* flags;
    const uint8_t* part;
    upart_t* upart;
    uint16_t* lite_cm;
    const uint32_t* crash_bits;
    const uint8_t* btab;
    Hdr* hdr;
    uint32_t *act, *pas;
    uint64_t *sentm, *recvm;
    uint64_t* mapx;
    uint32_t* mapx_top;
    uint32_t mapx_rows;
    uint32_t *pt_all, *pt_com, *pt_eag, *pt_laz, *pt_rt;
    uint32_t* conn;
    uint64_t* pt_out;
    uint64_t* outx;
    uint32_t* outx_top;
    uint32_t outx_rows;
    const uint32_t* origin;
    const uint32_t* slots;
    const uint32_t* in_beg;
    const unsigned long long* in_cb;
    const uint32_t* start;
    const uint4* desc;
    const uint32_t* n_alist;
    uint4* desc_slow;
    uint32_t* n_slow;
    uint4* desc_pt;
    uint32_t* n_pt;
    uint4* desc_shuf;
    uint32_t* n_shuf;
    uint64_t* stat_shuf;
    uint4* desc_lite;
    uint32_t* n_lite;
    uint64_t* stat_lite;
    uint4* desc_ptl;
    uint32_t* n_ptl;
    uint64_t* stat_ptl;
    uint64_t* stat_ptle;
    uint64_t* stat_relay;
    uint64_t* stat_pt;
    const Msg* rec_in;
    const uint64_t* obase;
    Msg* rec_out;
    uint32_t* okey;
    uint32_t* ocnt;
    uint64_t* stat_part;
    unsigned long long* ktime;
    const uint32_t* ctl;
    uint32_t pl, strategy, periodic, scamp_c, fanout;
    uint32_t fw;
    uint32_t tomb;
    uint32_t* fbits;
    const uint32_t* pay_in;
    uint32_t* pay_out;
    uint32_t* pay_top;
    uint32_t pay_cap;
    uint32_t* sview;
    uint32_t* sinv;
    uint32_t* stop_ids;
    uint32_t* n_stop;
    uint32_t faults, n_omit_s, n_omit_r;
    const uint8_t* faulted;
    const uint64_t* omit;
    const uint32_t* pay_imp;
    uint32_t imp_stride;
};
constexpr uint32_t PAY_IMPORT = 0x80000000u;

__global__ void k_consume(RoundArgs args);
constexpr uint32_t RELAY_MAX_BLOCKS = 8192;
constexpr uint32_t SHUF_MAX_BLOCKS = 1024;
#ifndef PSIM_PTL_BLOCK
#define PSIM_PTL_BLOCK 64
#endif
constexpr uint32_t PTL_BLOCK = PSIM_PTL_BLOCK;
__global__ void k_relay(RoundArgs args);
__global__ void k_consume_pl(RoundArgs args);
__global__ void k_shuf(RoundArgs args);
__global__ void k_consume_lite(RoundArgs args);
__global__ void k_lite_half(RoundArgs args);
__global__ void k_lite_quarter(RoundArgs args);
__global__ void k_hv_phase(RoundArgs args, uint32_t sgrid, uint32_t cgrid, uint32_t egrid);
struct LiteKernel {
    void (*kernel)(RoundArgs);
    uint32_t block;
    uint32_t grid_nodes;
    uint32_t resident;
    bool side_by_side;
};
LiteKernel lite_kernel_groups(bool half);
LiteKernel lite_kernel_wave();
enum : uint32_t { PTL_BOTH = 0, PTL_EARLY = 1, PTL_LATE = 2 };
__global__ void k_ptl(RoundArgs args);
__global__ void k_ptl_part(RoundArgs args, uint32_t part);
__global__ void k_pt(RoundArgs args);
int debug_stamps(unsigned long long* out);
int debug_stamps_half(unsigned long long* out);
uint32_t consume_grid();
uint32_t pt_grid();
uint32_t ptl_grid();

constexpr uint32_t CRASH_GRAIN_SHIFT = 4;
constexpr upart_t UPART_DOWN = (upart_t)(PSIM_UPART8 ? 0xFFu : 0x100u);
__device__ __forceinline__ bool crash_filter(const uint32_t* bits, uint32_t id) {
    const uint32_t g = id >> CRASH_GRAIN_SHIFT;
    return (bits[g >> 5] >> (g & 31)) & 1u;
}
template <class Args>
__device__ __forceinline__ bool crashed_now(Args& a, uint32_t id) {
    return crash_filter(a.crash_bits, id) && (a.flags[id] & F_CRASHED);
}

typedef const __attribute__((address_space(4))) RoundArgs KArgs;

template <class Args>
__device__ __forceinline__ uint4 ptl_desc(Args& a, const uint32_t (&c)[4], uint32_t i) {
    const uint32_t n = a.n_local;
    return a.desc_ptl[i < c[0] ? i
                    : i < c[0] + c[1] ? n - 1 - (i - c[0])
                    : i < c[0] + c[1] + c[2] ? n + (i - c[0] - c[1])
                    : 2 * n - 1 - (i - c[0] - c[1] - c[2])];
}
template <class Args>
__device__ __forceinline__ void ptl_counts(Args& a, uint32_t part, uint32_t (&c)[4], uint32_t& nq) {
    c[0] = part != PTL_LATE ? a.n_ptl[0] : 0u; c[1] = part != PTL_LATE ? a.n_ptl[1] : 0u;
    c[2] = part != PTL_EARLY ? a.n_ptl[2] : 0u; c[3] = part != PTL_EARLY ? a.n_ptl[3] : 0u;
    nq = c[0] + c[1] + c[2] + c[3];
}
template <class Args>
__device__ __forceinline__ uint32_t lite_at(Args& a, const uint32_t (&c)[4], uint32_t i) {
    const uint32_t n = a.n_local;
    return i < c[0] ? i
         : i < c[0] + c[1] ? n - 1 - (i - c[0])
         : i < c[0] + c[1] + c[2] ? n + (i - c[0] - c[1])
         : 2 * n - 1 - (i - c[0] - c[1] - c[2]);
}
template <class Args>
__device__ __forceinline__ void lite_counts(Args& a, uint32_t (&c)[4], uint32_t& na) {
    c[0] = a.n_lite[0]; c[1] = a.n_lite[1]; c[2] = a.n_lite[2]; c[3] = a.n_lite[3];
    na = c[0] + c[1] + c[2] + c[3];
}
#ifndef PSIM_SHORT_TAIL
#define PSIM_SHORT_TAIL 1
#endif

constexpr uint32_t layout_mix(uint32_t h, uint64_t v) {
    return ((h ^ (uint32_t)v) * 0x01000193u ^ (uint32_t)(v >> 32)) * 0x01000193u;
}
constexpr uint32_t layout_sig() {
    uint32_t h = 0x811C9DC5u;
    const uint64_t v[] = {
        PSIM_ABI_VERSION, sizeof(RoundArgs), offsetof(RoundArgs, flags), offsetof(RoundArgs, upart),
        offsetof(RoundArgs, relay_lead), sizeof(*RoundArgs().lite_cm),
        offsetof(RoundArgs, hdr), offsetof(RoundArgs, conn), offsetof(RoundArgs, outx_rows),
        offsetof(RoundArgs, desc), offsetof(RoundArgs, desc_lite), offsetof(RoundArgs, stat_ptle), offsetof(RoundArgs, stat_pt),
        offsetof(RoundArgs, rec_out), offsetof(RoundArgs, okey), offsetof(RoundArgs, ktime),
        offsetof(RoundArgs, ctl), offsetof(RoundArgs, fbits), offsetof(RoundArgs, omit), offsetof(RoundArgs, pay_imp),
        sizeof(Hdr), sizeof(Msg), sizeof(upart_t), PSIM_SHORT_TAIL, PTL_BLOCK, KEY_DST_BITS, KEY_BCAST,
        PSIM_ACTIVE_CAP, PSIM_PASSIVE_CAP, PSIM_EXCHANGE_CAP, PSIM_PT_ROOTS, PSIM_PT_OUT_CAP, PSIM_IDMAP_CAP,
        PSIM_CONN_CAP, PSIM_SVIEW_CAP, OUT_IN, IDMAP_IN, RT_SET, RT_WORDS, NST, CRASH_GRAIN_SHIFT};
    for (uint64_t x : v) h = layout_mix(h, x);
    return h;
}
uint32_t layout_sig_consume();
uint32_t layout_sig_lite();
uint32_t layout_sig_strategy();

inline uint32_t resident_grid(const void* kernel, uint32_t block) {
    int dev = 0, nb = 0;
    hipDeviceProp_t p;
    if (hipGetDevice(&dev) != hipSuccess || hipGetDeviceProperties(&p, dev) != hipSuccess ||
        hipOccupancyMaxActiveBlocksPerMultiprocessor(&nb, kernel, (int)block, 0) != hipSuccess || nb <= 0)
        return 1024;
    return (uint32_t)nb * (uint32_t)p.multiProcessorCount;
}

__device__ __forceinline__ KArgs& kargs() {
    KArgs* p = (KArgs*)__builtin_amdgcn_kernarg_segment_ptr();
    asm volatile("" : "+s"(p));
    return *p;
}

}
```

### partisan_amd/csrc/psim_lite.h

```cpp
#pragma once
#include <utility>

#include "psim_device.h"
#include "psim_kernels.h"
#include "psim_wave.h"

namespace psim {
namespace lite {
namespace {

#ifndef PSIM_HALF_WPB
#define PSIM_HALF_WPB 4
#endif
#ifndef PSIM_HALF_WAVES
#define PSIM_HALF_WAVES 4
#endif
#ifndef PSIM_QUARTER_WPB
#define PSIM_QUARTER_WPB 4
#endif
#ifndef PSIM_QUARTER_WAVES
#define PSIM_QUARTER_WAVES 4
#endif
#ifndef PSIM_LITE_ROWS_LDS
#define PSIM_LITE_ROWS_LDS 1
// ... 198 lines not shown
    uint32_t DCL, DCH;
};
constexpr uint32_t HF_PDIRTY = 16;
template <uint32_t W>
DEV uint32_t local_row(const Node<W>& x) { return x.me - kargs().lo; }
template <uint32_t W>
DEV uint32_t out_cap(const Node<W>& x) { return x.AF >> 8; }

template <uint32_t W>
DEV void dc_fill(Node<W>& x, uint64_t base) {
    const uint64_t v = draw58_at(base + Grp<W>::lane(), x.me, kargs().seed);
    x.DCL = (uint32_t)v; x.DCH = (uint32_t)(v >> 32);
    x.dcb = base;
}
template <uint32_t W>
DEV void dc_cover(Node<W>& x, uint64_t base, uint32_t n) {
    if (base < x.dcb || base + n > x.dcb + W) dc_fill(x, base);
}
template <uint32_t W>
DEV uint64_t draw(Node<W>& x) {
    using G = Grp<W>;
    const uint64_t c = x.rng++;
    dc_cover(x, c, 1);
    const uint32_t i = (uint32_t)(c - x.dcb);
    return ((uint64_t)G::get(x.DCH, i) << 32) | G::get(x.DCL, i);
}
template <uint32_t W>
DEV uint32_t uniform_n(Node<W>& x, const Lds<W>& w, uint32_t n) {
    const uint64_t two58 = 1ull << 58;
    const uint32_t M = Grp<W>::magic(w.KM, n);
    for (;;) {
        const uint64_t v = draw(x);
        if (v < n) return (uint32_t)v + 1;
        const uint32_t i = mod_small_m(v, n, M);
        if (v - i <= two58 - n) return i + 1;
    }
}

template <uint32_t W>
DEV uint32_t select_random(Node<W>& x, const Lds<W>& w, uint32_t V, uint32_t n, uint32_t o0, uint32_t o1) {
    using G = Grp<W>;
    const uint32_t l = G::lane();
    const uint32_t M = G::mask(l < n && V != o0 && V != o1);
    const uint32_t cnt = (uint32_t)__popc(M);
    if (cnt == 0) return PSIM_NONE;
    const uint32_t k = uniform_n(x, w, cnt) - 1;
    const bool hit = ((M >> l) & 1u) && (uint32_t)__popc(M & ((1u << l) - 1u)) == k;
    return G::get(V, (uint32_t)__ffs(G::mask(hit)) - 1);
}

template <int MAXN, uint32_t W>
DEV uint32_t sublist(Node<W>& x, Lds<W>& w, uint32_t V, uint32_t n, uint32_t k, uint32_t& OUT, uint32_t on) {
    using G = Grp<W>;
    static_assert(MAXN <= (int)W, "one entry and one cached draw a lane");
    const uint32_t l = G::lane();
    const uint64_t base = x.rng;
    dc_cover(x, base, n);
    const uint32_t src = (uint32_t)(base - x.dcb) + l;
    const uint64_t v = ((uint64_t)G::get(x.DCH, src) << 32) | G::get(x.DCL, src);
    const uint64_t key = l < n ? v >> 5 : ~0ull;
    const uint32_t m = n < k ? n : k;
    const uint32_t hi = (uint32_t)(key >> 21);
    uint32_t rank = 0;
    unroll<MAXN>([&](auto J) {
        const uint32_t hj = G::template getc<J>(hi);
        rank += hj < hi ? 1u : 0u;
        if constexpr (J % 8 == 7 && J + 1 < MAXN) __builtin_amdgcn_sched_barrier(0);
    });
    uint32_t* s = w.scr;
    if (l < n) s[rank] = l;
    __builtin_amdgcn_wave_barrier();
    const uint32_t owner = s[rank & 31];
    __builtin_amdgcn_wave_barrier();
    if (G::any(l < n && owner != l)) {
        rank = 0;
        for (uint32_t j = 0; j < n; j++) {
            const uint64_t kj = G::get64(key, j);
            const uint32_t ej = G::get(V, j);
            rank += (kj < key || (kj == key && ej < V)) ? 1u : 0u;
        }
    }
    if (l < n && rank < m) s[rank] = V;
    __builtin_amdgcn_wave_barrier();
    const uint32_t got = s[(l - on) & 31];
    __builtin_amdgcn_wave_barrier();
    OUT = (l >= on && l < on + m) ? got : OUT;
    x.rng = base + n;
    return on + m;
}
template <class Node>
DEV uint32_t Pas<32>::sublist(Node& x, Lds<32>& w, uint32_t k, uint32_t& OUT, uint32_t on) {
    return lite::sublist<PSIM_PASSIVE_CAP - 2>(x, w, x.pas.P, x.pas_n, k, OUT, on);
}
template <class Node>
DEV uint32_t Pas<16>::sublist(Node& x, Lds<16>& w, uint32_t k, uint32_t& OUT, uint32_t on) {
    const uint32_t P0 = x.pas.P0, P1 = x.pas.P1;
    const uint32_t l = G::lane(), n = x.pas_n, e0 = 2 * l, e1 = 2 * l + 1;
    const uint64_t base = x.rng;
    const uint64_t v0 = draw58_at(base + e0, x.me, kargs().seed);
    const uint64_t v1 = draw58_at(base + e1, x.me, kargs().seed);
    const uint64_t key0 = e0 < n ? v0 >> 5 : ~0ull, key1 = e1 < n ? v1 >> 5 : ~0ull;
    const uint32_t m = n < k ? n : k;
    const uint32_t hi0 = (uint32_t)(key0 >> 21), hi1 = (uint32_t)(key1 >> 21);
    uint32_t rank0 = 0, rank1 = 0;
    unroll<(PSIM_PASSIVE_CAP - 2) / 2>([&](auto J) {
        const uint32_t a = G::getc<J>(hi0), b = G::getc<J>(hi1);
        rank0 += (a < hi0 ? 1u : 0u) + (b < hi0 ? 1u : 0u);
        rank1 += (a < hi1 ? 1u : 0u) + (b < hi1 ? 1u : 0u);
    });
    uint32_t* s = w.scr;
    if (e0 < n) s[rank0] = e0;
    if (e1 < n) s[rank1] = e1;
    __builtin_amdgcn_wave_barrier();
    const uint32_t own0 = s[rank0 & 31], own1 = s[rank1 & 31];
    __builtin_amdgcn_wave_barrier();
    if (G::any((e0 < n && own0 != e0) || (e1 < n && own1 != e1))) {
        rank0 = 0; rank1 = 0;
        for (uint32_t j = 0; j < n; j++) {
            const uint64_t ks = (j & 1u) ? key1 : key0;
            const uint32_t es = (j & 1u) ? P1 : P0;
            const uint64_t kj = G::get64(ks, j >> 1);
            const uint32_t ej = G::get(es, j >> 1);
            rank0 += (kj < key0 || (kj == key0 && ej < P0)) ? 1u : 0u;
            rank1 += (kj < key1 || (kj == key1 && ej < P1)) ? 1u : 0u;
        }
    }
    if (e0 < n && rank0 < m) s[rank0] = P0;
    if (e1 < n && rank1 < m) s[rank1] = P1;
    __builtin_amdgcn_wave_barrier();
    const uint32_t got = s[(l - on) & 31];
    __builtin_amdgcn_wave_barrier();
    OUT = (l >= on && l < on + m) ? got : OUT;
    x.rng = base + n;
    return on + m;
}

template <uint32_t W>
DEV uint32_t usort(Lds<W>& w, uint32_t& E, bool valid) {
    using G = Grp<W>;
    const uint32_t l = G::lane();
    const uint32_t v = valid ? E : PSIM_NONE;
    bool dup = false;
    unroll<8>([&](auto J) {
        const uint32_t vj = G::template getc<J>(v);
        dup |= ((uint32_t)J < l) & (vj == v);
    });
    const uint32_t u = valid && !dup ? v : PSIM_NONE;
    uint32_t rank = 0;
    unroll<8>([&](auto J) {
        const uint32_t uj = G::template getc<J>(u);
        rank += uj < u ? 1u : 0u;
    });
    const uint32_t c = (uint32_t)__popc(G::mask(u != PSIM_NONE));
    uint32_t* s = w.scr;
    if (u != PSIM_NONE) s[rank] = u;
    __builtin_amdgcn_wave_barrier();
    const uint32_t got = s[l];
    __builtin_amdgcn_wave_barrier();
    E = l < c ? got : 0u;
    return c;
}

template <uint32_t W>
DEV void flush(Node<W>& x, Lds<W>& w) {
    using G = Grp<W>;
    const uint32_t l = G::lane();
    const uint32_t cnt = x.seq - x.flushed;
    const uint32_t cap = out_cap(x);
    __builtin_amdgcn_wave_barrier();
    for (uint32_t j0 = 0; j0 < cnt; j0 += G::FLUSH) {
        const uint32_t j = j0 + (l >> 2);
        if (j < cnt && x.flushed + j < cap)
            reinterpret_cast<uint4*>(kargs().rec_out + x.ob + x.flushed + j)[l & 3] =
                reinterpret_cast<const uint4*>(w.srec + j * 16)[l & 3];
    }
    if (l < cnt && x.flushed + l < cap) kargs().okey[x.ob + x.flushed + l] = w.skey[l];
    __builtin_amdgcn_wave_barrier();
    x.flushed = x.seq;
}

template <uint32_t W>
DEV void emit(Node<W>& x, Lds<W>& w, Cnt& c, uint32_t dst, uint32_t type, uint32_t ttl, uint32_t EX, uint32_t nex) {
    using G = Grp<W>;
    const uint32_t l = G::lane();
    const uint32_t k = x.seq - x.flushed;
    const uint32_t tt = type | (ttl << 8) | (nex << 16);
    const uint32_t exv = (uint32_t)__builtin_amdgcn_update_dpp(0, (int)EX, 0x118, 0xF, 0xF, true);
    const uint32_t word = l == 0 ? dst : l == 1 ? x.me : l == 2 ? tt : l == 3 ? x.seq
                        : l < 8 ? 0u : (l - 8 < nex ? exv : 0u);
    if (W == 16 || l < 16) {
        w.srec[k * 16 + l] = word;
        c.digest += (uint64_t)word * digest_mul(l);
    }
    if (l == 0) w.skey[k] = dst | (max_emit(type) << KEY_DST_BITS);
    x.seq++;
    c.em += type == PSIM_MSG_SHUFFLE ? 1u : 0x10000u;
    if (k + 1 == G::STAGE) flush(x, w);
}

template <uint32_t W>
DEV bool connect_ok(const Node<W>& x, uint32_t dst) {
    using G = Grp<W>;
    KArgs& a = kargs();
    if (dst >= a.n_nodes || dst == x.me) return false;
    const uint32_t m = G::mask(G::lane() < x.act_n && x.A == dst);
    if (m) return (x.AF >> (__ffs(m) - 1)) & 1u;
    return (uint32_t)a.upart[dst] == ((x.fl >> 8) & 0xFFu);
}

template <uint32_t W>
DEV void hv_send(Node<W>& x, Lds<W>& w, Cnt& c, uint32_t dst, uint32_t type, uint32_t ttl, uint32_t EX, uint32_t nex) {
    if (!connect_ok(x, dst)) { c.fail++; return; }
    x.rng++;
// ... 12 lines not shown
    bool in_act = false;
    unroll<PSIM_ACTIVE_CAP>([&](auto J) {
        const uint32_t aj = G::template getc<J>(AS);
        in_act |= aj == EX;
    });
    uint32_t T = EX;
    const bool valid = l < nex && EX != x.me && !in_act;
    uint32_t mt;
    if (PSIM_MERGE_SORTED && sorted) {
        const uint32_t vm = G::mask(valid);
        uint32_t* sc = w.scr;
        if (valid) sc[__popc(vm & ((1u << l) - 1u))] = EX;
        __builtin_amdgcn_wave_barrier();
        mt = (uint32_t)__popc(vm);
        const uint32_t got = sc[l];
        __builtin_amdgcn_wave_barrier();
        T = l < mt ? got : 0u;
    } else {
        mt = usort(w, T, valid);
    }
    if (!mt) return;
    const uint32_t maxp = a.max_passive;
    const uint8_t* bt = a.btab;
    Pas<W> pt = x.pas.tagged(bt, x.pas_n);
    const uint32_t TG = tag_of(bt, T, l < mt);
    const uint64_t c0 = x.rng;
    dc_cover(x, c0, mt);
    const uint32_t src = (uint32_t)(c0 - x.dcb) + l;
    const uint64_t v = ((uint64_t)G::get(x.DCH, src) << 32) | G::get(x.DCL, src);
    const uint32_t KI = mod_small_m(v, maxp, G::magic(w.KM, maxp));
    const bool par = !G::any(l < mt && v >= maxp && v - KI > (1ull << 58) - maxp);
    uint32_t used = 0, n = x.pas_n, dirty = 0;
    if (par) {
        uint32_t K = KI;
        uint32_t TT[PSIM_EXCHANGE_CAP];
        unroll<PSIM_EXCHANGE_CAP>([&](auto I) { TT[I] = G::template getc<I>(TG); });
        if constexpr (W == 32) __builtin_amdgcn_sched_barrier(0);
        unroll<PSIM_EXCHANGE_CAP>([&](auto I) {
            const uint32_t tt = TT[I];
            const bool mem = pt.has(tt);
            const bool ev = !mem && n >= maxp;
            const uint32_t k = G::get0(K);
            const uint32_t kn = G::next(K);
            K = ev ? kn : K;
            used += ev ? 1u : 0u;
            pt.step(n, dirty, tt, mem, ev, k);
        });
    } else {
        for (uint32_t i = 0; i < mt; i++) {
            const uint32_t tt = G::get(TG, i);
            const bool mem = pt.has(tt);
            if (mem) continue;
            const bool ev = n >= maxp;
            uint32_t k = 0;
            if (ev) {
                x.rng = c0 + used;
                k = uniform_n(x, w, n) - 1;
                used = (uint32_t)(x.rng - c0);
            }
            pt.step(n, dirty, tt, false, ev, k);
        }
    }
    x.pas_n = n;
    x.pas = pt.untagged();
    x.fl |= dirty ? HF_PDIRTY : 0u;
    x.rng = c0 + used;
}

#if PSIM_LITE_ROWS_LDS
#define PER_NODE(l) asm volatile("" : "+v"(l))
#else
#define PER_NODE(l) do { } while (0)
#endif
template <uint32_t W>
struct In {
    uint4 D;
    uint32_t r0, r1, w9, A, part;
    typename Pas<W>::Row P;
    uint32_t cm, oe;
    uint32_t SRC, TT;
    uint32_t EXP;
};

DEV uint4 load_desc(KArgs& a, const uint32_t (&lc)[4], uint32_t i, bool live) {
    return live ? a.desc_lite[lite_at(a, lc, i)] : make_uint4(0, 0, 0, 0);
}
template <uint32_t W>
DEV void load_rows(KArgs& a, In<W>& in, bool live) {
    const uint32_t l = Grp<W>::lane();
    const size_t li = live ? in.D.x - a.lo : 0;
    const uint32_t* hrow = reinterpret_cast<const uint32_t*>(a.hdr + li);
    in.r0 = hrow[0]; in.r1 = hrow[1]; in.w9 = hrow[9];
    in.A = l < PSIM_ACTIVE_CAP ? a.act[li * PSIM_ACTIVE_CAP + l] : 0u;
    in.P = Pas<W>::load(a.pas + li * PSIM_PASSIVE_CAP);
    in.part = a.part[live ? in.D.x : 0];
    in.cm = a.lite_cm[li];
    in.oe = reinterpret_cast<const uint32_t*>(a.obase + li + 1)[0];
}
#if PSIM_LITE_ROWS_LDS
template <uint32_t W>
struct Rows {
    static constexpr uint32_t X4 = 0, CM = 64 * 4, PT = CM + 64, WORDS = PT + 64;
    static constexpr uint32_t PAS = 0, ACT = 32, H0 = 40, H9 = 45, OE = 50, DESC = 52;
    static_assert(DESC + 4 <= W * 4, "a group's pieces: 14 lanes of its W");
};
typedef __attribute__((address_space(3))) void* lds_ptr_t;
typedef const __attribute__((address_space(1))) void* glb_ptr_t;
template <uint32_t W>
DEV void rows_table(KArgs& a, uint32_t* tab) {
    static_assert(PSIM_PASSIVE_CAP * 4 == 1 << 7 && PSIM_ACTIVE_CAP * 4 == 1 << 5 && sizeof(Hdr) == 1 << 6 &&
                  sizeof(*a.obase) == 1 << 3 && sizeof(*a.desc_lite) == 1 << 4, "the shifts below");
    for (uint32_t l = threadIdx.x; l < W; l += blockDim.x) {
        uint64_t b;
        uint32_t sh;
        if (l < 8) { b = (uint64_t)a.pas + l * 16; sh = 7; }
        else if (l < 10) { b = (uint64_t)a.act + (l - 8) * 16; sh = 5; }
        else if (l < 12) { b = (uint64_t)a.hdr + (l - 10) * 32; sh = 6; }
        else if (l < 13) { b = (uint64_t)a.obase; sh = 3; }
        else { b = (uint64_t)a.desc_lite; sh = 4; }
        tab[4 * l] = (uint32_t)b; tab[4 * l + 1] = (uint32_t)(b >> 32);
        tab[4 * l + 2] = sh; tab[4 * l + 3] = l < 13 ? 0u : 1u;
    }
}
template <uint32_t W>
DEV void rows_dma(KArgs& a, const Lds<W>& w, uint32_t lid, const uint4& D, bool live, uint32_t dn) {
    using R = Rows<W>;
    const uint32_t li = live ? D.x - a.lo : 0u;
    const uint4 t = reinterpret_cast<const uint4*>(w.tab)[lid & (W - 1)];
    const uint64_t src = (((uint64_t)t.y << 32) | t.x) + ((uint64_t)(t.w ? dn : li) << t.z);
    __builtin_amdgcn_global_load_lds((glb_ptr_t)src, (lds_ptr_t)(w.rows + R::X4), 16, 0, 0);
    __builtin_amdgcn_global_load_lds((glb_ptr_t)(a.lite_cm + li), (lds_ptr_t)(w.rows + R::CM), 2, 0, 0);
    __builtin_amdgcn_global_load_lds((glb_ptr_t)(a.part + (live ? D.x : 0u)), (lds_ptr_t)(w.rows + R::PT), 1, 0, 0);
}
template <uint32_t W>
DEV void rows_read(const Lds<W>& w, uint32_t lid, In<W>& in) {
    using R = Rows<W>;
    const uint32_t l = lid & (W - 1);
    const uint32_t* const g = w.rows + R::X4 + (lid & (64 - W)) * 4;
    in.r0 = g[R::H0]; in.r1 = g[R::H0 + 1]; in.w9 = g[R::H9];
    in.A = g[R::ACT + (l & (PSIM_ACTIVE_CAP - 1))];
    in.A = l < PSIM_ACTIVE_CAP ? in.A : 0u;
    in.P = reinterpret_cast<const typename Pas<W>::Row*>(g + R::PAS)[l];
    in.oe = g[R::OE];
    in.cm = w.rows[R::CM + lid] & 0xFFFFu;
    in.part = w.rows[R::PT + lid] & 0xFFu;
}

template <uint32_t W>
DEV uint4 desc_read(const Lds<W>& w, uint32_t lid, bool live) {
    using R = Rows<W>;
    const uint4 d = *reinterpret_cast<const uint4*>(w.rows + R::X4 + (lid & (64 - W)) * 4 + R::DESC);
    return live ? d : make_uint4(0, 0, 0, 0);
}
#endif
template <uint32_t W>
DEV In<W> load_in(KArgs& a, const uint4& D) {
    uint32_t l = Grp<W>::lane();
    PER_NODE(l);
    In<W> in;
    in.D = D;
    in.r0 = in.r1 = in.w9 = in.A = in.part = in.cm = in.oe = 0;
    in.P = {};
    const uint32_t ik = in.D.z & DESC_CNT_MASK;
    const Msg* r = a.rec_in + in.D.y + (l < ik ? l : 0u);
    const uint2 st = *reinterpret_cast<const uint2*>(&r->src);
    in.SRC = l < ik ? st.x : 0u;
    in.TT = l < ik ? st.y : (uint32_t)PSIM_MSG_PT_BROADCAST;
    in.EXP = a.rec_in[in.D.y + ((l >> 3) < ik ? (l >> 3) : 0u)].ex[l & 7];
// ... 30 lines not shown
      }
      uint32_t M = G::mask((TT & 0xFF) < PSIM_MSG_PT_BROADCAST);
      while (M) {
        const uint32_t j = (uint32_t)__ffs(M) - 1;
        M &= M - 1;
        const uint32_t p = G::get(SRC, j), tt = G::get(TT, j);
        const uint32_t ep = G::get(in.EXP, (j << 3) | (l & 7));
        const uint32_t q = cb + j;
        uint32_t ex = q < G::PREF ? ep : a.rec_in[x.ib + q].ex[l & 7];
        const uint32_t nex = (tt >> 16) & 0xFF, ttl = (tt >> 8) & 0xFF;
        const uint32_t type = tt & 0xFF;
        ex = l < nex ? ex : 0u;
        const bool reply = type == PSIM_MSG_SHUFFLE_REPLY;
        const bool relay = !reply && ttl > 0 && x.act_n > 1;
        c.dl += reply ? 0x10000u : 1u;
        LSTAMP(w, 6);
        if (relay) {
            const uint32_t r = select_random(x, w, x.A, x.act_n, p, x.me);
            if (r != PSIM_NONE) hv_send(x, w, c, r, PSIM_MSG_SHUFFLE, ttl - 1, ex, nex);
            LSTAMP(w, 1);
        } else {
            if (!reply) {
                uint32_t RESP = 0;
                const uint32_t nr = Pas<W>::sublist(x, w, nex, RESP, 0);
                LSTAMP(w, 2);
                hv_send(x, w, c, p, PSIM_MSG_SHUFFLE_REPLY, 0, RESP, nr);
                LSTAMP(w, 3);
            }
            merge_exchange(x, w, ex, nex, !reply);
            LSTAMP(w, 4);
        }
      }
    }
    if (x.fl & DESC_SHUFFLE) {
        uint32_t EX = l == 0 ? x.me : 0u;
        uint32_t m = 1;
        m = sublist<PSIM_ACTIVE_CAP>(x, w, x.A, x.act_n, a.k_active, EX, m);
        m = Pas<W>::sublist(x, w, a.k_passive, EX, m);
        const uint32_t nex = usort(w, EX, l < m);
        const uint32_t t = select_random(x, w, x.A, x.act_n, x.me, x.me);
        if (t != PSIM_NONE) hv_send(x, w, c, t, PSIM_MSG_SHUFFLE, a.arwl, EX, nex);
        LSTAMP(w, 5);
    }
}

template <uint32_t W>
DEV void count(Lds<W>& w, const Cnt& c) {
    if (Grp<W>::lane() != 0) return;
    unsigned long long* st = w.sst;
    if (c.pb & 0xFFFFu) atomicAdd(&st[ST_PROC], (unsigned long long)(c.pb & 0xFFFFu));
    if (c.pb >> 16) atomicAdd(&st[ST_BOUND], (unsigned long long)(c.pb >> 16));
    if (c.dl & 0xFFFFu) atomicAdd(&st[ST_DELIV + PSIM_MSG_SHUFFLE], (unsigned long long)(c.dl & 0xFFFFu));
    if (c.dl >> 16) atomicAdd(&st[ST_DELIV + PSIM_MSG_SHUFFLE_REPLY], (unsigned long long)(c.dl >> 16));
    if (c.em & 0xFFFFu) atomicAdd(&st[ST_EMIT + PSIM_MSG_SHUFFLE], (unsigned long long)(c.em & 0xFFFFu));
    if (c.em >> 16) atomicAdd(&st[ST_EMIT + PSIM_MSG_SHUFFLE_REPLY], (unsigned long long)(c.em >> 16));
    if (c.fail) atomicAdd(&st[ST_FAIL], (unsigned long long)c.fail);
}

template <uint32_t W>
DEV void writeback(Node<W>& x, Lds<W>& w, Cnt& c) {
    KArgs& a = kargs();
    const uint32_t l = Grp<W>::lane();
    const uint32_t li = local_row(x);
    uint32_t* hrow = reinterpret_cast<uint32_t*>(a.hdr + li);
    const uint32_t w9 = (x.fl & 0xFFFF0000u) | (x.pas_n << 8) | x.act_n;
    if (l < 3) hrow[l == 2 ? 9 : l] = l == 0 ? (uint32_t)x.rng : l == 1 ? (uint32_t)(x.rng >> 32) : w9;
    if (x.fl & HF_PDIRTY) x.pas.store(a.pas + (size_t)li * PSIM_PASSIVE_CAP);
    flush(x, w);
    if (l == 0) a.ocnt[li] = x.seq;
    c.pb += 1u + (x.seq > out_cap(x) ? 0x10000u : 0u);
    if ((c.dl | c.em | c.pb) & 0x80008000u) {
        count(w, c);
        c.dl = 0; c.em = 0; c.pb = 0; c.fail = 0;
    }
}

template <uint32_t W>
struct Carve {
    using G = Grp<W>;
    static constexpr uint32_t SREC = (NST * 2 + 3) & ~3u, SKEY = SREC + G::WPB * G::N * G::STAGE * 16,
                              SCR = SKEY + G::WPB * G::N * G::STAGE,
#if PSIM_LITE_ROWS_LDS
                              ROWS = SCR + G::WPB * G::N * G::SCR, TAB = ROWS + G::WPB * Rows<W>::WORDS,
                              WORDS = TAB + W * 4;
    static_assert(ROWS % 4 == 0 && TAB % 4 == 0, "the DMA's 16-B pieces, the table's 16-B entries");
#else
                              WORDS = SCR + G::WPB * G::N * G::SCR;
#endif
    static_assert(WORDS * 4 <= 40960, "the block's LDS: four blocks of it per CU at 4 waves/SIMD");
};
template <uint32_t W>
DEV void lite_kernel(const uint32_t bid, const uint32_t nblk, uint32_t* const pool) {
    using G = Grp<W>;
    constexpr uint32_t WPB = G::WPB, STAGE = G::STAGE;
    static_assert(STAGE >= 1 && STAGE <= 16, "flush writes a group's staged route keys one per lane");
    static_assert((STAGE * 16 * 4) % 16 == 0, "a group's staging area is read in 16-B pieces");
    static_assert(sizeof(Msg) == 16 * 4, "a record is one word per lane of a group's first row");
    static_assert(PSIM_PASSIVE_CAP == 32, "the passive row is one entry a lane of a half, two a lane of a row");
    static_assert(PSIM_ACTIVE_CAP <= 8 && PSIM_EXCHANGE_CAP == 8,
                  "a record's exchange ids move from lanes 0-7 to lanes 8-15 (row_shr:8)");
    static_assert(G::SCR >= PSIM_PASSIVE_CAP, "a sublist scatters one word per passive entry");
    static_assert(WPB * G::N * (STAGE * 16 + STAGE + G::SCR) * 4 + NST * 8 <= 64 * 1024,
                  "the block's LDS: four blocks of it per CU at 4 waves/SIMD");
    if (*kargs().ctl) return;
    unsigned long long* const sst = reinterpret_cast<unsigned long long*>(pool);
    uint32_t* const srecs = pool + Carve<W>::SREC;
    uint32_t* const skeys = pool + Carve<W>::SKEY;
    uint32_t* const scrs = pool + Carve<W>::SCR;
#ifdef PSIM_STAMPS
    __shared__ unsigned long long stls[WPB][32];
    for (int i = threadIdx.x; i < (int)(WPB * 32); i += blockDim.x) (&stls[0][0])[i] = 0;
#endif
    for (int i = threadIdx.x; i < NST; i += blockDim.x) sst[i] = 0;
#if PSIM_LITE_ROWS_LDS
    rows_table<W>(kargs(), pool + Carve<W>::TAB);
#endif
    __syncthreads();
    const uint32_t wid = threadIdx.x >> 6, g = G::idx();
    Lds<W> w;
    w.sst = sst;
    w.srec = srecs + (wid * G::N + g) * (STAGE * 16);
    w.skey = skeys + (wid * G::N + g) * STAGE;
    w.scr = scrs + (wid * G::N + g) * G::SCR;
    w.KM = G::magic_lanes();
#ifdef PSIM_STAMPS
    w.stl = stls[wid];
    w.t_last = __builtin_amdgcn_s_memtime();
#endif
    Cnt c = {};
    const uint32_t nw = nblk * WPB;
    const uint32_t first = G::N * (bid * WPB + wid) + g;
    const uint32_t step = G::N * nw;
    uint32_t lc[4], na;
    lite_counts(kargs(), lc, na);
#if PSIM_LITE_ROWS_LDS
    for (uint32_t k = 0; k < 4; k++) lc[k] = (uint32_t)__builtin_amdgcn_readfirstlane((int)lc[k]);
    na = lc[0] + lc[1] + lc[2] + lc[3];
    w.rows = pool + Carve<W>::ROWS + (uint32_t)__builtin_amdgcn_readfirstlane((int)wid) * Rows<W>::WORDS;
    w.tab = pool + Carve<W>::TAB;
    if (first < na) {
        Node<W> x;
        In<W> in = load_in<W>(kargs(), load_desc(kargs(), lc, first, true));
        rows_dma(kargs(), w, __lane_id(), in.D, true, lite_at(kargs(), lc, first + step < na ? first + step : first));
        asm volatile("s_waitcnt vmcnt(0)" ::: "memory");
        uint4 Dn = desc_read(w, __lane_id(), first + step < na);
        for (uint32_t i = first; i < na; i += step) {
            LSTAMP(w, 8);
            uint32_t lid = __lane_id();
            PER_NODE(lid);
            rows_read(w, lid, in);
            begin(x, in);
            x.AF = (in.cm & 0xFFu) | (min(in.oe - x.ob, 0xFFFFFFu) << 8);
            const uint32_t nx = i + step, nnx = i + 2 * step;
            In<W> inn = load_in<W>(kargs(), Dn);
            asm volatile("s_waitcnt lgkmcnt(0)" ::: "memory");
            rows_dma(kargs(), w, lid, Dn, nx < na, lite_at(kargs(), lc, nnx < na ? nnx : i));
            LSTAMP(w, 0);
            body(x, w, c, in);
            LSTAMP(w, 9);
            asm volatile("s_waitcnt vmcnt(0)" ::: "memory");
            asm volatile("" : "+v"(inn.SRC), "+v"(inn.TT), "+v"(inn.EXP));
            Dn = desc_read(w, lid, nnx < na);
            writeback(x, w, c);
            LSTAMP(w, 7);
            in = inn;
        }
        count(w, c);
    }
#else
    if (first < na) {
        Node<W> x;
        In<W> in = load_in<W>(kargs(), load_desc(kargs(), lc, first, true));
        load_rows(kargs(), in, true);
        uint4 Dn = load_desc(kargs(), lc, first + step < na ? first + step : first, first + step < na);
        for (uint32_t i = first; i < na; i += step) {
            LSTAMP(w, 8);
            begin(x, in);
            x.AF = (in.cm & 0xFFu) | (min(in.oe - x.ob, 0xFFFFFFu) << 8);
            const uint32_t nx = i + step, nnx = i + 2 * step;
            In<W> inn = load_in<W>(kargs(), Dn);
            LSTAMP(w, 0);
            body(x, w, c, in);
            LSTAMP(w, 9);
            Dn = load_desc(kargs(), lc, nnx < na ? nnx : i, nnx < na);
            load_rows(kargs(), inn, nx < na);
            writeback(x, w, c);
            LSTAMP(w, 7);
            in = inn;
        }
        count(w, c);
    }
#endif
    {
        uint64_t dg = c.digest;
#pragma unroll
        for (int off = 32; off > 0; off >>= 1) dg += __shfl_xor(dg, off);
        if (__lane_id() == 0 && dg) atomicAdd(&sst[ST_DIGEST], (unsigned long long)dg);
    }
    __syncthreads();
    for (int i = threadIdx.x; i < NST; i += blockDim.x)
        kargs().stat_lite[(size_t)bid * NST + i] = sst[i];
#ifdef PSIM_STAMPS
    if (threadIdx.x < 32) {
        unsigned long long t = 0;
        for (uint32_t k = 0; k < WPB; k++) t += stls[k][threadIdx.x];
        if (t) atomicAdd(&g_stamps_half[threadIdx.x], t);
    }
#endif
}

}
}
}
```

### partisan_amd/sim.py

```python
import ctypes as C

import numpy as np

from . import _abi
from .workloads import NONE


class SimError(RuntimeError):
    rc = None


def default_config(**kw):
    cfg = _abi.PsimConfig()
    cfg.abi_version = _abi.PSIM_ABI_VERSION
    cfg.n_nodes = 32
    cfg.seed = 1
    cfg.max_active_size, cfg.min_active_size, cfg.max_passive_size = 6, 3, 30
    cfg.arwl, cfg.prwl, cfg.k_active, cfg.k_passive = 5, 30, 3, 4
    cfg.shuffle_period, cfg.promotion_period, cfg.random_promotion = 10, 5, 1
    cfg.persist_epoch, cfg.plumtree, cfg.lazy_tick_period = 0, 1, 1
    cfg.device, cfg.n_shards, cfg.shard_rank, cfg.shard_world = -1, 1, 0, 1
    cfg.comm_id = None
    cfg.max_msgs_per_round = 0
    cfg.manager, cfg.strategy = _abi.MANAGER_HYPARVIEW, _abi.STRATEGY_FULL
# ... 366 lines not shown
        out = {}
        for name, _ in _abi.PsimResilience._fields_:
            if name == "reserved":
                continue
            v = getattr(m, name)
            out[name] = np.array(v[:], np.uint64) if hasattr(v, "__len__") else int(v)
        return out

    def gossip_reach(self, sources, fanouts, thresholds=None, salts=None, fail_seed=0, max_levels=0):
        src = np.ascontiguousarray(sources, np.uint32).reshape(-1)
        cols = [src, np.ascontiguousarray(fanouts, np.uint32).reshape(-1)]
        for v in (thresholds, salts):
            cols.append(np.zeros(src.size, np.uint32) if v is None else np.ascontiguousarray(v, np.uint32).reshape(-1))
        if any(c.size != src.size for c in cols):
            raise ValueError("sources, fanouts, thresholds and salts differ in length")
        cases = (_abi.PsimGossipCase * max(src.size, 1))()
        for j in range(src.size):
            cases[j].source, cases[j].fanout, cases[j].threshold, cases[j].salt = (int(c[j]) for c in cols)
        m = _abi.PsimGossipReach()
        self._check(self._extra["get_gossip_reach"](self._h, cases if src.size else None, src.size, int(fail_seed),
                                                    max_levels, C.byref(m)), "get_gossip_reach")
        out = {}
        for name, _ in _abi.PsimGossipReach._fields_:
            if name == "reserved":
                continue
            v = getattr(m, name)
            out[name] = np.array(v[:], np.uint64) if hasattr(v, "__len__") else int(v)
        return out

    def relay_reach(self, sources, targets, ttls, max_levels=0):
        src = np.ascontiguousarray(sources, np.uint32).reshape(-1)
        dst = np.ascontiguousarray(targets, np.uint32).reshape(-1)
        ttl = np.full(src.size, ttls, np.uint32) if np.ndim(ttls) == 0 else np.ascontiguousarray(ttls, np.uint32).reshape(-1)
        if not src.size == dst.size == ttl.size:
            raise ValueError("sources, targets and ttls differ in length")
        cases = (_abi.PsimRelayCase * max(src.size, 1))()
        for j in range(src.size):
            cases[j].source, cases[j].target, cases[j].ttl = int(src[j]), int(dst[j]), int(ttl[j])
        m = _abi.PsimRelayReach()
        self._check(self._extra["get_relay_reach"](self._h, cases if src.size else None, src.size, max_levels,
                                                   C.byref(m)), "get_relay_reach")
        out = {}
        for name, _ in _abi.PsimRelayReach._fields_:
            if name == "reserved":
                continue
            v = getattr(m, name)
            out[name] = np.array(v[:], np.uint64) if hasattr(v, "__len__") else int(v)
        return out

    def trace_watch(self, nodes=None, to=True, frm=True, types=None, capacity=1 << 20):
        mask = (1 << _abi.NTYPES) - 1
        if types is not None:
            mask = 0
            for t in types:
                mask |= 1 << int(t)
        d = (_abi.PSIM_TRACE_TO if to else 0) | (_abi.PSIM_TRACE_FROM if frm else 0)
        if nodes is None:
            ptr, n = None, 0
        else:
            ids = np.ascontiguousarray(nodes, np.uint32).reshape(-1)
            ptr, n = _abi.u32p(ids), ids.size
        self._check(self._extra["trace_watch"](self._h, ptr, n, d, mask & 0xFFFFFFFF, capacity), "trace_watch")

    def trace_read(self):
        n, lost = C.c_size_t(), C.c_uint64()
        self._check(self._extra["trace_read"](self._h, None, None, 0, C.byref(n), C.byref(lost)), "trace_read")
        recs = np.zeros((n.value, 16), np.uint32)
        rounds = np.zeros(n.value, np.uint32)
        self._check(self._extra["trace_read"](self._h, _abi.u32p(recs), _abi.u32p(rounds), n.value, C.byref(n),
                                              C.byref(lost)), "trace_read")
        return recs, rounds, lost.value

    def trace_clear(self):
        self._check(self._extra["trace_clear"](self._h), "trace_clear")

    KERNELS = ("k_relay", "k_shuf", "k_lite_half", "k_consume", "k_ptl", "k_pt", "k_node_prep")

    def kernel_counts(self):
        out = (C.c_uint64 * 28)()
        k = self._extra["debug_kernel_counts"](self._h, out, 28)
        self._check(min(k, 0), "debug_kernel_counts")
        return {self.KERNELS[i]: (out[4 * i], out[4 * i + 1], out[4 * i + 2]) for i in range(k)}

    def kernel_times(self):
        cap = 64
        names = (C.c_char_p * cap)()
        ms = (C.c_double * cap)()
        launches = (C.c_uint64 * cap)()
        k = self._extra["kernel_times"](self._h, names, ms, launches, cap)
        return {names[i].decode(): (ms[i], launches[i]) for i in range(k)}


class HostSim(Simulator):

    def __init__(self, cfg, lo, hi):
        from . import _lib

        self.lo, self.hi = lo, hi
        self._host = _abi.bind(_lib.load(), "psim_", _abi.HOST_BOUNDARY)
        super().__init__(cfg, comm=host_comm_id(lo, hi))

    def emit(self):
        self._check(self._host["round_emit"](self._h), "round_emit")

    def outbound(self):
        n = C.c_size_t()
        self._check(self._host["get_outbound"](self._h, None, 0, C.byref(n)), "get_outbound")
        out = np.zeros((n.value, 16), np.uint32)
        self._check(self._host["get_outbound"](self._h, _abi.u32p(out), n.value, C.byref(n)), "get_outbound")
        return out

    def absorb(self, recs):
        r = np.ascontiguousarray(recs, np.uint32).reshape(-1, 16)
        st = np.zeros(1, _abi.STATS_DTYPE)
        self._check(self._host["round_absorb"](self._h, _abi.u32p(r), r.shape[0],
                                                st.ctypes.data_as(C.POINTER(_abi.PsimRoundStats))), "round_absorb")
        return st

    def nodes(self, first=None, count=None):
        first = self.lo if first is None else first
        return super().nodes(first, self.hi - first if count is None else count)

    def strategy_nodes(self, first=None, count=None):
        first = self.lo if first is None else first
        return super().strategy_nodes(first, self.hi - first if count is None else count)


__all__ = ["Simulator", "HostSim", "SimError", "default_config", "comm_id", "host_comm_id", "NONE"]
```

Measured before the change: 3.273 billion.

## Bin lite-path nodes by fine message-sequence key to reduce wave divergence

The relay kernel now classifies each lite node by a small key built from the types and order of its first messages (term, relay-led, mixed, shuffle due). It counts the key into per-bin LDS counters and scatters descriptors into many lite bins instead of four. The lite consume kernels build a per-block prefix table in LDS and walk bins through a cursor, so nodes processed together by a wave follow the same message sequence. This costs extra LDS atomics, a larger descriptor array and a prefix-table setup per block. It is enabled by default only when PSIM_LITE_BINS selects the fine count and the shard is at or below the node cap.

```diff
diff --git a/include/partisan_gpu_sim.h b/include/partisan_gpu_sim.h
--- a/include/partisan_gpu_sim.h
+++ b/include/partisan_gpu_sim.h
@@ -415,6 +415,8 @@
 
 int psim_debug_kernel_counts(psim_handle *h, uint64_t *out, int cap);
 
+int psim_debug_lite_list(psim_handle *h, uint32_t *ids, uint32_t *bins, int cap, int *n);
+
 int psim_kernel_times(psim_handle *h, const char **names, double *ms, uint64_t *launches, int cap);
 
 int psim_get_exchange_stats(psim_handle *h, uint64_t *records, uint64_t *bytes);
diff --git a/partisan_amd/_abi.py b/partisan_amd/_abi.py
--- a/partisan_amd/_abi.py
+++ b/partisan_amd/_abi.py
@@ -271,6 +271,7 @@
     "restore": (C.c_int, [_H, C.c_void_p, C.c_size_t]),
     "get_exchange_stats": (C.c_int, [_H, C.POINTER(C.c_uint64), C.POINTER(C.c_uint64)]),
     "debug_kernel_counts": (C.c_int, [_H, C.POINTER(C.c_uint64), C.c_int]),
+    "debug_lite_list": (C.c_int, [_H, _P32, _P32, C.c_int, C.POINTER(C.c_int)]),
     "get_strategy_histograms": (C.c_int, [_H, C.POINTER(PsimStrategyHistograms)]),
     "get_graph_metrics": (C.c_int, [_H, _P32, C.c_size_t, C.c_uint32, C.POINTER(PsimGraphMetrics)]),
     "get_tree_metrics": (C.c_int, [_H, C.c_uint32, C.c_uint32, C.POINTER(PsimTreeMetrics)]),
diff --git a/partisan_amd/csrc/psim_consume.hip b/partisan_amd/csrc/psim_consume.hip
--- a/partisan_amd/csrc/psim_consume.hip
+++ b/partisan_amd/csrc/psim_consume.hip
@@ -1568,7 +1568,9 @@
     __shared__ uint32_t scratch[LITE_WPB][64];
     __shared__ __attribute__((aligned(16))) uint32_t srecs[LITE_WPB][STAGE * 16];
     __shared__ uint32_t skeys[LITE_WPB][STAGE];
+    __shared__ uint32_t lpre[LITE_PRE_WORDS];
     for (int i = threadIdx.x; i < NST; i += blockDim.x) sst[i] = 0;
+    lite_table(kargs(), lpre);
     __syncthreads();
     const uint32_t wid = threadIdx.x >> 6;
     const uint32_t gw = uni(blockIdx.x * LITE_WPB + wid);
@@ -1591,15 +1593,14 @@
     w.SC = 0;
     w.digest = 0;
     w.KM = magic_lanes();
-    uint32_t lc[4], na;
-    lite_counts(kargs(), lc, na);
+    const uint32_t na = uni(lpre[LITE_BINS]), nl = kargs().n_local;
+    LiteCursor cb = lite_cursor(lpre);
     if (gw < na) {
         const uint32_t last = na - 1;
-        KArgs& a0 = kargs();
-        NodeIn x = load_node<false>(a0, reinterpret_cast<const uint32_t*>(kargs().desc_lite + lite_at(a0, lc, gw))[lane_id() & 3]);
+        NodeIn x = load_node<false>(kargs(), reinterpret_cast<const uint32_t*>(kargs().desc_lite + lite_at(lpre, nl, cb, gw))[lane_id() & 3]);
         NodeX y = load_x<true>(kargs(), x);
-        NodeIn xn = load_node<false>(kargs(), reinterpret_cast<const uint32_t*>(kargs().desc_lite + lite_at(a0, lc, min(gw + nw, last)))[lane_id() & 3]);
-        uint32_t d = reinterpret_cast<const uint32_t*>(kargs().desc_lite + lite_at(a0, lc, min(gw + 2 * nw, last)))[lane_id() & 3];
+        NodeIn xn = load_node<false>(kargs(), reinterpret_cast<const uint32_t*>(kargs().desc_lite + lite_at(lpre, nl, cb, min(gw + nw, last)))[lane_id() & 3]);
+        uint32_t d = reinterpret_cast<const uint32_t*>(kargs().desc_lite + lite_at(lpre, nl, cb, min(gw + 2 * nw, last)))[lane_id() & 3];
         for (uint32_t i = gw; i < na; i += nw) {
             STAMP(w, 0);
             begin_node(w, x, y);
@@ -1609,7 +1610,7 @@
             writeback_lite(w);
             STAMP(w, 10);
             NodeIn xnn = load_node<false>(kargs(), d);
-            d = reinterpret_cast<const uint32_t*>(kargs().desc_lite + lite_at(kargs(), lc, min(i + 3 * nw, last)))[lane_id() & 3];
+            d = reinterpret_cast<const uint32_t*>(kargs().desc_lite + lite_at(lpre, nl, cb, min(i + 3 * nw, last)))[lane_id() & 3];
             x = xn; y = yn; xn = xnn;
             STAMP(w, 11);
         }
@@ -1881,16 +1882,16 @@
 #ifndef PSIM_PTL_BIN
 #define PSIM_PTL_BIN 1
 #endif
-#ifndef PSIM_LITE_BIN
-#define PSIM_LITE_BIN 1
-#endif
+enum : uint32_t { KS_SEEN = 3u, KS_K1 = 1u << 2, KS_K2_SHIFT = 3, KS_LEAD = 1u << 5, KS_TERM = 1u << 6, KS_RELAY = 1u << 7 };
 __global__ void __launch_bounds__(256, PSIM_RELAY_WAVES) k_relay(RoundArgs) {
     if (*kargs().ctl) return;
     if (blockIdx.x == 0 && threadIdx.x == 0) kargs().ktime[0] = __builtin_amdgcn_s_memrealtime();
     enum { R_PROC, R_DELIV, R_SHUF, R_FAIL, R_DIGEST, R_BOUND, R_DELIV_FJ, R_FJ, R_N };
     __shared__ unsigned long long sst[R_N];
-    __shared__ uint32_t wc5[11][5];
+    __shared__ uint32_t wc5[7][5];
+    __shared__ uint32_t lcn[LITE_BINS], lbs[LITE_BINS];
     if (threadIdx.x < R_N) sst[threadIdx.x] = 0;
+    if (threadIdx.x < LITE_BINS) lcn[threadIdx.x] = 0;
     __syncthreads();
     const uint32_t l = lane_id();
     const uint32_t na = *kargs().n_alist;
@@ -1901,8 +1902,8 @@
         KArgs& a = kargs();
         const uint32_t P = base + threadIdx.x;
         uint4 D = make_uint4(0, 0, 0, 0);
-        bool heavy = false, to_pt = false, relay = false, maps = false, shuf = false, lite = false, bcast = false, term = false,
-             extra = false;
+        bool heavy = false, to_pt = false, relay = false, maps = false, shuf = false, lite = false, bcast = false;
+        uint32_t ks = 0;
         Hdr h;
         uint32_t ik = 0, oend = 0;
         uint4 act0 = make_uint4(0, 0, 0, 0), act1 = act0;
@@ -1926,7 +1927,7 @@
             hvm = 0;
             bool all_relay = true, all_shuf = true, term_out = false, fjn = false;
             uint32_t nf = ~0u;
-            bcast = false; term = false; extra = (tf & DESC_SHUFFLE) != 0;
+            bcast = false;
             const uint32_t av[8] = {act0.x, act0.y, act0.z, act0.w, act1.x, act1.y, act1.z, act1.w};
             for (uint32_t j = 0; j < ik; j += 4) {
                 uint2 T[4];
@@ -1951,9 +1952,12 @@
                         fjn |= fj;
                         all_relay &= (type == PSIM_MSG_SHUFFLE && ttl > 0) || fj;
                         all_shuf &= type == PSIM_MSG_SHUFFLE || type == PSIM_MSG_SHUFFLE_REPLY;
-                        term |= type == PSIM_MSG_SHUFFLE && !relays;
-                        extra |= type == PSIM_MSG_SHUFFLE && relays;
-                        nf = type == PSIM_MSG_SHUFFLE && relays ? nf : min(nf, j + q);
+                        const bool rel = type == PSIM_MSG_SHUFFLE && relays;
+                        nf = rel ? nf : min(nf, j + q);
+                        const uint32_t kind = rel ? 3u : type == PSIM_MSG_SHUFFLE ? 1u : 2u, sn = ks & KS_SEEN;
+                        ks |= type == PSIM_MSG_SHUFFLE ? (rel ? KS_RELAY : KS_TERM) : 0u;
+                        ks = sn == 0 ? ks | (rel ? KS_LEAD : 1u | (kind == 2u ? KS_K1 : 0u))
+                           : sn == 1 ? (ks + 1u) | (kind << KS_K2_SHIFT) : ks | KS_SEEN;
                         if (type == PSIM_MSG_SHUFFLE && !relays) {
                             bool in = false;
 #pragma unroll
@@ -2029,44 +2033,58 @@
             const bool ptl = P < na && to_pt && !origin_node, lt = P < na && lite;
             const bool pe = ptl && (!a.ptl_split || (!heavy && !lite && !shuf)), pl = ptl && !pe;
             const bool pb = bcast || !PSIM_PTL_BIN;
-            const bool lt0 = lt && !(extra && PSIM_LITE_BIN), lt1 = lt && extra && PSIM_LITE_BIN;
-            const bool tb = term || !PSIM_LITE_BIN;
-            const bool g[11] = {P < na && heavy, P < na && to_pt && origin_node, pe && pb,
-                                P < na && shuf, lt0 && tb, pe && !pb, lt0 && !tb,
-                                lt1 && tb, lt1 && !tb, pl && pb, pl && !pb};
-            uint64_t m[11];
-#pragma unroll
-            for (int k = 0; k < 11; k++) m[k] = ballot(g[k]);
+            {
+                const uint32_t due = (D.z >> 28) & DESC_SHUFFLE ? 1u : 0u;
+                const uint32_t more = (ks & KS_SEEN) == KS_SEEN || ((ks & KS_LEAD) && !first) ? 1u : 0u;
+                ks = a.lite_fine ? ((ks >> 2) & 7u) | (more << 3) | (due << 4)
+                                 : ((ks & KS_TERM) ? 0u : 1u) | ((ks & KS_RELAY) || due ? 2u : 0u);
+            }
+            const bool g[7] = {P < na && heavy, P < na && to_pt && origin_node, pe && pb,
+                               P < na && shuf, pe && !pb, pl && pb, pl && !pb};
+            uint64_t m[7];
+#pragma unroll
+            for (int k = 0; k < 7; k++) m[k] = ballot(g[k]);
             const uint32_t wv = threadIdx.x >> 6, nwv = blockDim.x >> 6;
             __syncthreads();
             if (l == 0)
 #pragma unroll
-                for (int k = 0; k < 11; k++) wc5[k][wv] = popc(m[k]);
+                for (int k = 0; k < 7; k++) wc5[k][wv] = popc(m[k]);
+            if (lt) ks |= atomicAdd(&lcn[ks], 1u) << 5;
             __syncthreads();
-            if (threadIdx.x < 11) {
-                const uint32_t k = threadIdx.x;
+            if (threadIdx.x < 64) {
+                uint32_t k = threadIdx.x;
+                asm volatile("" : "+v"(k));
+                const uint32_t b = k & (LITE_BINS - 1);
                 uint32_t t = 0;
-                for (uint32_t j = 0; j < nwv; j++) t += wc5[k][j];
+                if (k < 7)
+                    for (uint32_t j = 0; j < nwv; j++) t += wc5[k][j];
+                else if (k >= 32) {
+                    t = lcn[b];
+                    lcn[b] = 0;
+                }
                 uint32_t* cnt = k == 0 ? a.n_slow : k == 1 ? a.n_pt : k == 2 ? a.n_ptl : k == 3 ? a.n_shuf
-                              : k == 4 ? a.n_lite : k == 5 ? a.n_ptl + 1 : k < 9 ? a.n_lite + (k - 5)
-                              : a.n_ptl + (k - 7);
-                wc5[k][4] = t ? atomicAdd(cnt, t) : 0u;
+                              : k < 7 ? a.n_ptl + (k - 3) : a.n_lite + b;
+                const uint32_t at0 = t ? atomicAdd(cnt, t) : 0u;
+                if (k < 7) wc5[k][4] = at0;
+                else if (k >= 32) lbs[b] = at0;
             }
             __syncthreads();
-#pragma unroll
-            for (int k = 0; k < 11; k++)
+            const uint32_t nl = a.n_local;
+#pragma unroll
+            for (int k = 0; k < 7; k++)
                 if (g[k]) {
                     uint32_t b0 = wc5[k][4];
                     for (uint32_t j = 0; j < wv; j++) b0 += wc5[k][j];
                     const uint32_t at = b0 + popc(m[k] & lt_mask());
-                    uint4* desc = k == 0 ? a.desc_slow : k == 1 ? a.desc_pt : k == 2 || k == 5 || k >= 9 ? a.desc_ptl
-                                : k == 3 ? a.desc_shuf : a.desc_lite;
-                    const uint32_t nl = a.n_local;
-                    desc[k == 5 || k == 6 ? nl - 1 - at : k == 7 || k == 9 ? nl + at
-                         : k == 8 || k == 10 ? 2 * nl - 1 - at : at] =
-                        k == 0 && maps ? make_uint4(D.x, D.y, D.z | DESC_MAPS_BIT, D.w)
-                        : k == 4 || (k >= 6 && k <= 8) ? make_uint4(D.x, D.y + first, D.z - first, D.w) : D;
+                    uint4* desc = k == 0 ? a.desc_slow : k == 1 ? a.desc_pt : k == 3 ? a.desc_shuf : a.desc_ptl;
+                    desc[k == 4 ? nl - 1 - at : k == 5 ? nl + at : k == 6 ? 2 * nl - 1 - at : at] =
+                        k == 0 && maps ? make_uint4(D.x, D.y, D.z | DESC_MAPS_BIT, D.w) : D;
                 }
+            if (lt) {
+                const uint32_t lbin = ks & (LITE_BINS - 1), at = lbs[lbin] + (ks >> 5);
+                a.desc_lite[(size_t)(lbin >> 1) * nl + ((lbin & 1u) ? nl - 1 - at : at)] =
+                    make_uint4(D.x, D.y + first, D.z - first, D.w);
+            }
         }
         if (P >= na || heavy) continue;
         const uint32_t id = D.x;
diff --git a/partisan_amd/csrc/psim_engine.hip b/partisan_amd/csrc/psim_engine.hip
--- a/partisan_amd/csrc/psim_engine.hip
+++ b/partisan_amd/csrc/psim_engine.hip
@@ -1291,7 +1291,7 @@
     if (blockIdx.x == 0 && threadIdx.x == 0) {
         a.ktime[0] = ~0ull; a.ktime[1] = 0; *a.n_slow = 0; *a.n_pt = 0;
         if (a.n_shuf) *a.n_shuf = 0;
-        if (a.n_lite) { a.n_lite[0] = 0; a.n_lite[1] = 0; a.n_lite[2] = 0; a.n_lite[3] = 0; }
+        if (a.n_lite) for (uint32_t k = 0; k < LITE_BINS; k++) a.n_lite[k] = 0;
         if (a.n_ptl) { a.n_ptl[0] = 0; a.n_ptl[1] = 0; a.n_ptl[2] = 0; a.n_ptl[3] = 0; }
         if (a.n_stop) *a.n_stop = 0;
     }
@@ -1485,7 +1485,7 @@
             ctl[2] = 0;
             a.ktime[0] = ~0ull; a.ktime[1] = 0; *a.n_slow = 0; *a.n_pt = 0;
             if (a.n_shuf) *a.n_shuf = 0;
-            if (a.n_lite) { a.n_lite[0] = 0; a.n_lite[1] = 0; a.n_lite[2] = 0; a.n_lite[3] = 0; }
+            if (a.n_lite) for (uint32_t k = 0; k < LITE_BINS; k++) a.n_lite[k] = 0;
             if (a.n_ptl) { a.n_ptl[0] = 0; a.n_ptl[1] = 0; a.n_ptl[2] = 0; a.n_ptl[3] = 0; }
             if (a.n_stop) *a.n_stop = 0;
         }
@@ -1637,6 +1637,26 @@
         return e && *e ? atoi(e) != 0 : RELAY_LEAD_DEFAULT != 0;
     }();
     return v;
+}
+
+constexpr uint32_t LITE_FINE_NODES = 1u << 22;
+constexpr int LITE_BINS_DEFAULT = 4;
+bool lite_fine_shard(uint32_t n) {
+    static const bool fine = [] {
+        const char* e = getenv("PSIM_LITE_BINS");
+        int v = e && *e ? atoi(e) : LITE_BINS_DEFAULT;
+        if (v != 4 && v != (int)LITE_BINS) {
+            std::fprintf(stderr, "psim: PSIM_LITE_BINS=%s is neither 4 nor %u: using %d\n", e, LITE_BINS, LITE_BINS_DEFAULT);
+            v = LITE_BINS_DEFAULT;
+        }
+        return v == (int)LITE_BINS;
+    }();
+    static const uint32_t cap = [] {
+        const char* e = getenv("PSIM_LITE_BINS_NODES");
+        const unsigned long v = e && *e ? strtoul(e, nullptr, 10) : LITE_FINE_NODES;
+        return (uint32_t)std::min<unsigned long>(v, LITE_FINE_NODES);
+    }();
+    return fine && n <= cap;
 }
 
 constexpr int PREP_FUSED_DEFAULT = 1;
@@ -1696,6 +1716,7 @@
     a.xbot = c.manager == PSIM_MANAGER_XBOT; a.xbot_period = c.xbot_period;
     a.ptl_split = ptl_early_knob() != 0;
     a.relay_lead = relay_lead_knob() && h->lite.kernel != psim::k_consume_lite;
+    a.lite_fine = lite_fine_shard(s->n);
     a.strategy = c.strategy; a.periodic = c.periodic_interval; a.scamp_c = c.scamp_c;
     a.fanout = c.fanout; a.fw = h->fw; a.tomb = h->tomb;
     a.fbits = s->fbits.p; a.sview = s->sview.p; a.sinv = s->sinv.p;
@@ -2537,7 +2558,7 @@
             std::fprintf(stderr, "psim: round %llu shard %u: %u nodes with work, %u to k_consume, %u to k_pt, "
                          "%u to k_shuf, %u to k_consume_lite, %u to k_ptl, outbox bound %llu, emitted %llu\n",
                          (unsigned long long)h->round, s->idx, read1(s, s->d_nact.p), read1(s, s->n_slow.p),
-                         read1(s, s->n_pt.p), read1(s, s->n_shuf.p), read1(s, s->n_lite.p) + read1(s, s->n_lite.p + 1) + read1(s, s->n_lite.p + 2) + read1(s, s->n_lite.p + 3),
+                         read1(s, s->n_pt.p), read1(s, s->n_shuf.p), [&] { uint32_t t = 0; for (uint32_t k = 0; k < LITE_BINS; k++) t += read1(s, s->n_lite.p + k); return t; }(),
                          read1(s, s->n_ptl.p) + read1(s, s->n_ptl.p + 1) + read1(s, s->n_ptl.p + 2) + read1(s, s->n_ptl.p + 3),
                          (unsigned long long)s->pin[PIN_TOTAL], (unsigned long long)em);
         }
@@ -3079,7 +3100,7 @@
     rc |= s->desc_slow.alloc(n); rc |= s->n_slow.alloc(1);
     rc |= s->desc_pt.alloc(n); rc |= s->n_pt.alloc(1);
     rc |= s->desc_shuf.alloc(n); rc |= s->n_shuf.alloc(1);
-    rc |= s->desc_lite.alloc(2 * n); rc |= s->n_lite.alloc(4);
+    rc |= s->desc_lite.alloc((lite_fine_shard((uint32_t)n) ? LITE_BINS / 2 : 2) * (size_t)n); rc |= s->n_lite.alloc(LITE_BINS);
     rc |= s->desc_ptl.alloc(2 * n); rc |= s->n_ptl.alloc(4);
     if (h->cfg.manager == PSIM_MANAGER_PLUGGABLE) { rc |= s->stop_ids.alloc(n); rc |= s->n_stop.alloc(1); }
     rc |= s->stat_out.alloc(STAT_OUT_N);
@@ -4192,6 +4213,30 @@
     return nk;
 }
 
+int psim_debug_lite_list(psim_handle* h, uint32_t* ids, uint32_t* bins, int cap, int* n) {
+    if (!h || !ids || !bins || !n || cap < 0) return PSIM_EINVAL;
+    *n = 0;
+    if (h->cfg.manager == PSIM_MANAGER_PLUGGABLE) return PSIM_OK;
+    Shard* s = h->shards[0];
+    HIP_TRY(hipStreamSynchronize(s->stream));
+    uint32_t cnt[LITE_BINS];
+    HIP_TRY(hipMemcpy(cnt, s->n_lite.p, sizeof cnt, hipMemcpyDeviceToHost));
+    const size_t arrays = s->desc_lite.n / s->n;
+    std::vector<uint4> run;
+    int at = 0;
+    for (uint32_t b = 0; b < LITE_BINS; b++) {
+        if (!cnt[b]) continue;
+        if (b / 2 >= arrays || cnt[b] > s->n) return PSIM_EDEVICE;
+        run.resize(cnt[b]);
+        const size_t from = (size_t)(b / 2) * s->n + ((b & 1) ? s->n - cnt[b] : 0);
+        HIP_TRY(hipMemcpy(run.data(), s->desc_lite.p + from, (size_t)cnt[b] * sizeof(uint4), hipMemcpyDeviceToHost));
+        for (uint32_t j = 0; j < cnt[b]; j++, at++)
+            if (at < cap) { ids[at] = run[j].x; bins[at] = b; }
+    }
+    *n = at;
+    return PSIM_OK;
+}
+
 int psim_debug_stamps(unsigned long long* out, int cap) {
     if (!out || cap < 96) return PSIM_EINVAL;
     return psim::debug_stamps(out);
diff --git a/partisan_amd/csrc/psim_kernels.h b/partisan_amd/csrc/psim_kernels.h
--- a/partisan_amd/csrc/psim_kernels.h
+++ b/partisan_amd/csrc/psim_kernels.h
@@ -23,6 +23,7 @@
     uint32_t xbot, xbot_period;
     uint32_t ptl_split;
     uint32_t relay_lead;
+    uint32_t lite_fine;
     uint32_t crash_round, tracked_msg;
     uint32_t upart_dirty;
     uint32_t lazy_wake;
@@ -155,18 +156,40 @@
     c[2] = part != PTL_EARLY ? a.n_ptl[2] : 0u; c[3] = part != PTL_EARLY ? a.n_ptl[3] : 0u;
     nq = c[0] + c[1] + c[2] + c[3];
 }
-template <class Args>
-__device__ __forceinline__ uint32_t lite_at(Args& a, const uint32_t (&c)[4], uint32_t i) {
-    const uint32_t n = a.n_local;
-    return i < c[0] ? i
-         : i < c[0] + c[1] ? n - 1 - (i - c[0])
-         : i < c[0] + c[1] + c[2] ? n + (i - c[0] - c[1])
-         : 2 * n - 1 - (i - c[0] - c[1] - c[2]);
-}
-template <class Args>
-__device__ __forceinline__ void lite_counts(Args& a, uint32_t (&c)[4], uint32_t& na) {
-    c[0] = a.n_lite[0]; c[1] = a.n_lite[1]; c[2] = a.n_lite[2]; c[3] = a.n_lite[3];
-    na = c[0] + c[1] + c[2] + c[3];
+constexpr uint32_t LITE_BINS = 32;
+constexpr uint32_t LITE_PRE_WORDS = 36;
+template <class Args>
+__device__ __forceinline__ void lite_table(Args& a, uint32_t* pre) {
+    if (threadIdx.x < 64) {
+        const uint32_t l = threadIdx.x;
+        uint32_t c = l < LITE_BINS ? a.n_lite[l] : 0u;
+#pragma unroll
+        for (uint32_t off = 1; off < LITE_BINS; off <<= 1) {
+            const uint32_t t = __shfl_up(c, off);
+            c += l >= off ? t : 0u;
+        }
+        if (l < LITE_BINS) pre[l + 1] = c;
+        if (l == 0) pre[0] = 0;
+    }
+}
+struct LiteCursor {
+    uint32_t b, lo, hi;
+};
+__device__ __forceinline__ LiteCursor lite_cursor(const uint32_t* pre) {
+    return LiteCursor{0u, 0u, (uint32_t)__builtin_amdgcn_readfirstlane((int)pre[1])};
+}
+__device__ __forceinline__ uint32_t lite_at(const uint32_t* pre, uint32_t n, LiteCursor& c, uint32_t i) {
+    uint32_t b = c.b, lo = c.lo, hi = c.hi;
+    while (i >= hi && b < LITE_BINS - 1) {
+        b++;
+        lo = hi;
+        hi = pre[b + 1];
+    }
+    c.b = (uint32_t)__builtin_amdgcn_readfirstlane((int)b);
+    c.lo = (uint32_t)__builtin_amdgcn_readfirstlane((int)lo);
+    c.hi = (uint32_t)__builtin_amdgcn_readfirstlane((int)hi);
+    const uint32_t k = min(i - lo, n - 1);
+    return (b >> 1) * n + ((b & 1u) ? n - 1 - k : k);
 }
 #ifndef PSIM_SHORT_TAIL
 #define PSIM_SHORT_TAIL 1
@@ -179,7 +202,7 @@
     uint32_t h = 0x811C9DC5u;
     const uint64_t v[] = {
         PSIM_ABI_VERSION, sizeof(RoundArgs), offsetof(RoundArgs, flags), offsetof(RoundArgs, upart),
-        offsetof(RoundArgs, relay_lead), sizeof(*RoundArgs().lite_cm),
+        offsetof(RoundArgs, relay_lead), offsetof(RoundArgs, lite_fine), LITE_BINS, sizeof(*RoundArgs().lite_cm),
         offsetof(RoundArgs, hdr), offsetof(RoundArgs, conn), offsetof(RoundArgs, outx_rows),
         offsetof(RoundArgs, desc), offsetof(RoundArgs, desc_lite), offsetof(RoundArgs, stat_ptle), offsetof(RoundArgs, stat_pt),
         offsetof(RoundArgs, rec_out), offsetof(RoundArgs, okey), offsetof(RoundArgs, ktime),
diff --git a/partisan_amd/csrc/psim_lite.h b/partisan_amd/csrc/psim_lite.h
--- a/partisan_amd/csrc/psim_lite.h
+++ b/partisan_amd/csrc/psim_lite.h
@@ -304,7 +304,9 @@
     }
     if (l < n && rank < m) s[rank] = V;
     __builtin_amdgcn_wave_barrier();
-    const uint32_t got = s[(l - on) & 31];
+    uint32_t lo = l;
+    asm volatile("" : "+v"(lo));
+    const uint32_t got = s[(lo - on) & 31];
     __builtin_amdgcn_wave_barrier();
     OUT = (l >= on && l < on + m) ? got : OUT;
     x.rng = base + n;
@@ -350,7 +352,9 @@
     if (e0 < n && rank0 < m) s[rank0] = P0;
     if (e1 < n && rank1 < m) s[rank1] = P1;
     __builtin_amdgcn_wave_barrier();
-    const uint32_t got = s[(l - on) & 31];
+    uint32_t lo = l;
+    asm volatile("" : "+v"(lo));
+    const uint32_t got = s[(lo - on) & 31];
     __builtin_amdgcn_wave_barrier();
     OUT = (l >= on && l < on + m) ? got : OUT;
     x.rng = base + n;
@@ -529,8 +533,9 @@
     uint32_t EXP;
 };
 
-DEV uint4 load_desc(KArgs& a, const uint32_t (&lc)[4], uint32_t i, bool live) {
-    return live ? a.desc_lite[lite_at(a, lc, i)] : make_uint4(0, 0, 0, 0);
+DEV uint4 load_desc(KArgs& a, const uint32_t* pre, LiteCursor& cb, uint32_t i, bool live) {
+    const uint32_t at = lite_at(pre, a.n_local, cb, i);
+    return live ? a.desc_lite[at] : make_uint4(0, 0, 0, 0);
 }
 template <uint32_t W>
 DEV void load_rows(KArgs& a, In<W>& in, bool live) {
@@ -727,11 +732,12 @@
                               SCR = SKEY + G::WPB * G::N * G::STAGE,
 #if PSIM_LITE_ROWS_LDS
                               ROWS = SCR + G::WPB * G::N * G::SCR, TAB = ROWS + G::WPB * Rows<W>::WORDS,
-                              WORDS = TAB + W * 4;
+                              PRE = TAB + W * 4;
     static_assert(ROWS % 4 == 0 && TAB % 4 == 0, "the DMA's 16-B pieces, the table's 16-B entries");
 #else
-                              WORDS = SCR + G::WPB * G::N * G::SCR;
-#endif
+                              PRE = SCR + G::WPB * G::N * G::SCR;
+#endif
+    static constexpr uint32_t WORDS = PRE + LITE_PRE_WORDS;
     static_assert(WORDS * 4 <= 40960, "the block's LDS: four blocks of it per CU at 4 waves/SIMD");
 };
 template <uint32_t W>
@@ -760,6 +766,8 @@
 #if PSIM_LITE_ROWS_LDS
     rows_table<W>(kargs(), pool + Carve<W>::TAB);
 #endif
+    const uint32_t* const pre = pool + Carve<W>::PRE;
+    lite_table(kargs(), pool + Carve<W>::PRE);
     __syncthreads();
     const uint32_t wid = threadIdx.x >> 6, g = G::idx();
     Lds<W> w;
@@ -776,30 +784,29 @@
     const uint32_t nw = nblk * WPB;
     const uint32_t first = G::N * (bid * WPB + wid) + g;
     const uint32_t step = G::N * nw;
-    uint32_t lc[4], na;
-    lite_counts(kargs(), lc, na);
+    const uint32_t na = (uint32_t)__builtin_amdgcn_readfirstlane((int)pre[LITE_BINS]);
+    LiteCursor cb = lite_cursor(pre);
 #if PSIM_LITE_ROWS_LDS
-    for (uint32_t k = 0; k < 4; k++) lc[k] = (uint32_t)__builtin_amdgcn_readfirstlane((int)lc[k]);
-    na = lc[0] + lc[1] + lc[2] + lc[3];
     w.rows = pool + Carve<W>::ROWS + (uint32_t)__builtin_amdgcn_readfirstlane((int)wid) * Rows<W>::WORDS;
     w.tab = pool + Carve<W>::TAB;
     if (first < na) {
         Node<W> x;
-        In<W> in = load_in<W>(kargs(), load_desc(kargs(), lc, first, true));
-        rows_dma(kargs(), w, __lane_id(), in.D, true, lite_at(kargs(), lc, first + step < na ? first + step : first));
+        In<W> in = load_in<W>(kargs(), load_desc(kargs(), pre, cb, first, true));
+        rows_dma(kargs(), w, __lane_id(), in.D, true, lite_at(pre, kargs().n_local, cb, min(first + step, na - 1)));
         asm volatile("s_waitcnt vmcnt(0)" ::: "memory");
         uint4 Dn = desc_read(w, __lane_id(), first + step < na);
         for (uint32_t i = first; i < na; i += step) {
             LSTAMP(w, 8);
+            const uint32_t nx = i + step, nnx = i + 2 * step;
+            const uint32_t dn = lite_at(pre, kargs().n_local, cb, min(nnx, na - 1));
             uint32_t lid = __lane_id();
             PER_NODE(lid);
             rows_read(w, lid, in);
             begin(x, in);
             x.AF = (in.cm & 0xFFu) | (min(in.oe - x.ob, 0xFFFFFFu) << 8);
-            const uint32_t nx = i + step, nnx = i + 2 * step;
             In<W> inn = load_in<W>(kargs(), Dn);
             asm volatile("s_waitcnt lgkmcnt(0)" ::: "memory");
-            rows_dma(kargs(), w, lid, Dn, nx < na, lite_at(kargs(), lc, nnx < na ? nnx : i));
+            rows_dma(kargs(), w, lid, Dn, nx < na, dn);
             LSTAMP(w, 0);
             body(x, w, c, in);
             LSTAMP(w, 9);
@@ -815,9 +822,9 @@
 #else
     if (first < na) {
         Node<W> x;
-        In<W> in = load_in<W>(kargs(), load_desc(kargs(), lc, first, true));
+        In<W> in = load_in<W>(kargs(), load_desc(kargs(), pre, cb, first, true));
         load_rows(kargs(), in, true);
-        uint4 Dn = load_desc(kargs(), lc, first + step < na ? first + step : first, first + step < na);
+        uint4 Dn = load_desc(kargs(), pre, cb, min(first + step, na - 1), first + step < na);
         for (uint32_t i = first; i < na; i += step) {
             LSTAMP(w, 8);
             begin(x, in);
@@ -827,7 +834,7 @@
             LSTAMP(w, 0);
             body(x, w, c, in);
             LSTAMP(w, 9);
-            Dn = load_desc(kargs(), lc, nnx < na ? nnx : i, nnx < na);
+            Dn = load_desc(kargs(), pre, cb, min(nnx, na - 1), nnx < na);
             load_rows(kargs(), inn, nx < na);
             writeback(x, w, c);
             LSTAMP(w, 7);
diff --git a/partisan_amd/sim.py b/partisan_amd/sim.py
--- a/partisan_amd/sim.py
+++ b/partisan_amd/sim.py
@@ -472,6 +472,14 @@
         self._check(min(k, 0), "debug_kernel_counts")
         return {self.KERNELS[i]: (out[4 * i], out[4 * i + 1], out[4 * i + 2]) for i in range(k)}
 
+    def lite_list(self):
+        cap = int(self.cfg.n_nodes)
+        ids = (C.c_uint32 * cap)()
+        bins = (C.c_uint32 * cap)()
+        n = C.c_int(0)
+        self._check(self._extra["debug_lite_list"](self._h, ids, bins, cap, C.byref(n)), "debug_lite_list")
+        return [(int(ids[i]), int(bins[i])) for i in range(min(n.value, cap))]
+
     def kernel_times(self):
         cap = 64
         names = (C.c_char_p * cap)()
diff --git a/profiles/lite_bins/order_model.py b/profiles/lite_bins/order_model.py
--- /dev/null
+++ b/profiles/lite_bins/order_model.py
@@ -0,0 +1,40 @@
+import os
+import sys
+
+ROOT = os.path.dirname(os.path.dirname(os.path.dirname(os.path.abspath(__file__))))
+sys.path.insert(0, ROOT)
+sys.path.insert(0, os.path.join(ROOT, "tests"))
+
+import _lite_bins_cases as B
+
+
+def main():
+    sizes = [int(a) for a in sys.argv[1:]] or [4096, 16384, 65536]
+    rows = []
+    for n in sizes:
+        _, _, keys = B.survey_reference(n)
+        total, distinct, seqs, pure4, pure_fine, cost = B.model_table(keys)
+        g = p = 0
+        for r, k in keys.items():
+            if r >= B.SURVEY_BOOT and k:
+                alt = {i: (v[0], (0 if "T" in v[2] else 1) | (2 if ("r" in v[2] or "+S" in v[2]) else 0), v[2])
+                       for i, v in k.items()}
+                a, b = B.pure_groups(alt, 1)
+                g, p = g + a, p + b
+        rows.append((n, total, distinct, pure4, pure_fine, cost, p / max(g, 1)))
+        print("== %d nodes: %d lite-like node-rounds, %d of %d fine keys occur ==" % (n, total, distinct, B.FINE_BINS))
+        rest = 0
+        for s, c in sorted(seqs.items(), key=lambda kv: -kv[1]):
+            if c * 100.0 / total >= 1.0:
+                print("  %-6s %5.1f %%" % (s, c * 100.0 / total))
+            else:
+                rest += c
+        print("  others %5.1f %%" % (rest * 100.0 / total))
+    print("nodes    groups of four with one sequence: four bins   (leading relays not counted as extra)   fine key"
+          "   lockstep cost fine / four")
+    for n, _, _, pure4, pure_fine, cost, alt4 in rows:
+        print("%-8d %38.1f %% %30.1f %% %14.1f %% %12.2f" % (n, 100 * pure4, 100 * alt4, 100 * pure_fine, cost))
+
+
+if __name__ == "__main__":
+    main()
```

Result: slower. 3.223 billion (-1.5%).
